# HLLMR/stratum-dsp

Measured on AMD Instinct MI355X. Metric: tracks/sec full analyze_audio(), 3-min 44.1 kHz mono, at 1/2/4/8 MI355X, higher is better.
Workload: dtype f32

## Files before the change

### stratum-dsp_amd/csrc/k_hpcp.hip

```cpp
#include "block_utils.hpp"
#include "kernels.hpp"

namespace sdsp {

constexpr int HP_CW = 16;
constexpr int HPB_CW = HP_CW;
static_assert(HPB_CW == 16, "k_hpcp_band stages a chunk as four 16-byte groups per row");
constexpr int HP_HU = 4;

template <int KCAP>
struct HpcpFrame {
    float e = 0.0f, m1 = 0.0f, m2 = 0.0f;
    float thr = -1.0f;
    float pm[KCAP];
    int pb[KCAP];
    __device__ __forceinline__ void init() {
#pragma unroll
        for (int q = 0; q < KCAP; q++) {
            pm[q] = -1.0f;
            pb[q] = 0;
        }
    }
    template <bool ENERGY = true>
    __device__ __forceinline__ void walk(const float* row, int c0, int cw, const HpcpParams& P) {
        for (int j = 0; j < cw; j++) {
            const int b = c0 + j;
            const float m = row[j];
            if (ENERGY) e += m * m;
            const int c = b - 1;
            if (c >= P.pk_lo && c <= P.pk_hi && !(m1 <= m2 || m1 < m) && m1 > thr) {
                bool gt[KCAP];
#pragma unroll
                for (int q = 0; q < KCAP; q++) gt[q] = m1 > pm[q];
#pragma unroll
                for (int q = KCAP - 1; q >= 1; q--) {
                    const int nbv = gt[q - 1] ? pb[q - 1] : c;
                    pm[q] = __builtin_amdgcn_fmed3f(pm[q], m1, pm[q - 1]);
                    pb[q] = gt[q] ? nbv : pb[q];
                }
                pm[0] = gt[0] ? m1 : pm[0];
                pb[0] = gt[0] ? c : pb[0];
                thr = pm[KCAP - 1];
            }
            m2 = m1;
            m1 = m;
        }
    }
    __device__ __forceinline__ void finish(float (*pc)[HP_FRAMES], int i, const HpcpParams& P,
                                           const HarmEntry* __restrict__ harm, float* __restrict__ chroma,
                                           float* __restrict__ energy, uint64_t g) {
#pragma unroll
        for (int q = 0; q < 12; q++) pc[q][i] = 0.0f;
#pragma unroll
        for (int k = 0; k < KCAP; k++) {
            if (k >= P.K || !(pm[k] > 0.0f)) continue;
            const int bin = pb[k];
            const float xk = sd_maxf(pm[k], 0.0f);
            float w0;
            if (P.p == 0.5f) {
                const float s = __builtin_sqrtf(xk);
                w0 = sd_sqrt_is_powf_half(xk, s) ? s : sd_powf_ool(xk, 0.5f);
            } else {
                w0 = sd_powf_ool(xk, P.p);
            }
            if (w0 <= 0.0f) continue;
            HarmEntry hv[HP_HU];
#pragma unroll
            for (int h = 0; h < HP_HU; h++)
                if (h < P.hmax) hv[h] = harm[bin * HP_HMAX + h];
            bool stop = false;
#pragma unroll
            for (int h = 0; h < HP_HU; h++) {
                if (stop || h >= P.hmax) break;
                const HarmEntry& he = hv[h];
                if (he.state == 0) {
                    stop = true;
                    break;
                }
                if (he.state == 1) continue;
                const float contrib = w0 * he.hw;
                for (int o = 0; o < 3; o++) pc[he.tc[o]][i] += contrib * he.wt[o];
            }
            for (int h = HP_HU + 1; !stop && h <= P.hmax; h++) {
                const HarmEntry he = harm[bin * HP_HMAX + (h - 1)];
                if (he.state == 0) break;
                if (he.state == 1) continue;
                const float contrib = w0 * he.hw;
                for (int o = 0; o < 3; o++) pc[he.tc[o]][i] += contrib * he.wt[o];
            }
        }
        float nsq = 0.0f;
#pragma unroll
        for (int q = 0; q < 12; q++) nsq += pc[q][i] * pc[q][i];
        const float norm = __builtin_sqrtf(nsq);
#pragma unroll
        for (int q = 0; q < 12; q++) {
            float v = pc[q][i];
            if (norm > EPS) v /= norm;
            chroma[g * 12 + q] = v;
        }
        energy[g] = e;
    }
};

template <int KCAP>
__global__ __launch_bounds__(HP_FRAMES) __attribute__((amdgpu_waves_per_eu(4))) void k_hpcp(const float* __restrict__ mags,
                                                    const uint64_t* __restrict__ frame_pfx,
                                                    const uint64_t* __restrict__ tile_pfx,
                                                    const int* __restrict__ tracks, int n_items, HpcpParams P,
                                                    const HarmEntry* __restrict__ harm, float* __restrict__ chroma,
                                                    float* __restrict__ energy) {
    __shared__ float tile[HP_FRAMES][HP_CW + 1];
    __shared__ float pcs[12][HP_FRAMES];
    const uint64_t gb = blockIdx.x;
    const int it = find_track(tile_pfx, n_items, gb);
    const int trk = tracks[it];
    const int64_t F = (int64_t)(frame_pfx[trk + 1] - frame_pfx[trk]);
    const int64_t f0 = (int64_t)(gb - tile_pfx[it]) * HP_FRAMES;
    const int i = threadIdx.x;
    const int64_t f = f0 + i;
    const bool valid = f < F;
    const int lane = i & 63, wrow = i & ~63;
    const int64_t rows = F - f0 < HP_FRAMES ? F - f0 : HP_FRAMES;
    if (wrow >= rows) return;
    const uint64_t g0 = frame_pfx[trk];
    HpcpFrame<KCAP> hf;
    hf.init();
    constexpr int RSTEP = 64 / HP_CW;
    constexpr int NLD = 64 / RSTEP;
    const int sub = lane / HP_CW, jj = lane % HP_CW;
    const float* rowp = mags + (g0 + (uint64_t)f0 + (uint64_t)(wrow + sub)) * (uint64_t)P.stride + jj;
    const uint64_t rstride = (uint64_t)RSTEP * (uint64_t)P.stride;
    float nx[NLD];
    auto load_chunk = [&](int c0) {
        const bool col_ok = c0 + jj < P.B;
#pragma unroll
        for (int u = 0; u < NLD; u++)
            nx[u] = (wrow + sub + u * RSTEP < rows && col_ok) ? rowp[(uint64_t)u * rstride + c0] : 0.0f;
    };
    auto wave_sync = [] {
        __builtin_amdgcn_fence(__ATOMIC_RELEASE, "wavefront");
        __builtin_amdgcn_wave_barrier();
        __builtin_amdgcn_fence(__ATOMIC_ACQUIRE, "wavefront");
    };
    load_chunk(0);
    for (int c0 = 0; c0 < P.B; c0 += HP_CW) {
        wave_sync();
#pragma unroll
        for (int u = 0; u < NLD; u++) tile[wrow + sub + u * RSTEP][jj] = nx[u];
        wave_sync();
        if (c0 + HP_CW < P.B) load_chunk(c0 + HP_CW);
        if (!valid) continue;
        hf.walk(tile[i], c0, P.B - c0 < HP_CW ? P.B - c0 : HP_CW, P);
    }
    if (!valid) return;
    hf.finish(pcs, i, P, harm, chroma, energy, g0 + (uint64_t)f);
}

__device__ float energy_delta(const float* __restrict__ pp, uint64_t total, int n_blocks, int B, float e_blk) {
    if (!(e_blk > 0.0f)) return 0.0f;
    const double u = 0x1p-24, g63 = 63.0 * u / (1.0 - 63.0 * u), g64 = 64.0 * u / (1.0 - 64.0 * u);
    const double gN = (double)B * u / (1.0 - (double)B * u), iu = 1.0 / (1.0 - g63);
    double pu = 0.0, pt = 0.0, eref = 0.0, eo = 0.0;
    for (int g = 0; g < n_blocks; g++) {
        const double bt = (double)pp[(uint64_t)g * total], bu = bt * iu;
        pu += bu;
        pt += bt;
        const int nb = B - 64 * g < 64 ? B - 64 * g : 64;
        eref += __builtin_fmin(bu, (double)nb * u * (1.0 + u) * pu * (1.0 + gN));
        eo += pt;
    }
    const double D = (eref + u * (1.0 + u) * (1.0 + g64) * eo + g63 * pu) * (1.0 + 1e-9);
    const double r = D / (double)e_blk;
    if (!(r < 1.0)) return 1.0f;
    float d = (float)r;
    if ((double)d < r) d = __uint_as_float(__float_as_uint(d) + 1u);
    return d;
}

constexpr float KC_IU_F = (float)(1.0 / (1.0 - 63.0 * 0x1p-24 / (1.0 - 63.0 * 0x1p-24)));
__device__ float energy_delta_f32(float e_blk, float pu, float eref, float eo, const float* __restrict__ pp,
                                  uint64_t total, int n_blocks, int B) {
    if (!(e_blk > 0.0f)) return 0.0f;
    if (!(e_blk >= 0x1p-60f && e_blk <= 0x1p100f)) return energy_delta(pp, total, n_blocks, B, e_blk);
    const float u = 0x1p-24f;
    const float g63 = 63.0f * u / (1.0f - 63.0f * u), g64 = 64.0f * u / (1.0f - 64.0f * u);
    const float D = eref + u * (1.0f + u) * (1.0f + g64) * eo + g63 * pu;
    const float r = (D / e_blk) * (1.0f + 0x1p-14f);
    if (!(r < 1.0f)) return 1.0f;
    return r;
}

template <int KCAP>
__global__ __launch_bounds__(HP_FRAMES) __attribute__((amdgpu_waves_per_eu(4))) void k_hpcp_band(const float* __restrict__ mags,
                                                         const uint64_t* __restrict__ frame_pfx,
                                                         const uint64_t* __restrict__ tile_pfx,
                                                         const int* __restrict__ tracks, int n_items, HpcpParams P,
                                                         const HarmEntry* __restrict__ harm,
                                                         const float* __restrict__ part, int n_blocks, uint64_t total,
                                                         float* __restrict__ chroma, float* __restrict__ energy,
                                                         float* __restrict__ edel) {
    __shared__ float tile[HP_FRAMES][HPB_CW + 1];
    __shared__ float pcs[12][HP_FRAMES];
    const uint64_t gb = blockIdx.x;
    const int it = find_track(tile_pfx, n_items, gb);
    const int trk = tracks[it];
    const int64_t F = (int64_t)(frame_pfx[trk + 1] - frame_pfx[trk]);
    const int64_t f0 = (int64_t)(gb - tile_pfx[it]) * HP_FRAMES;
    const int i = threadIdx.x;
    const int64_t f = f0 + i;
    const bool valid = f < F;
    const int lane = i & 63, wrow = i & ~63;
    const int64_t rows = F - f0 < HP_FRAMES ? F - f0 : HP_FRAMES;
    if (wrow >= rows) return;
    const uint64_t g0 = frame_pfx[trk];
    HpcpFrame<KCAP> hf;
    hf.init();
    if (valid) {
        const float* pp = part + g0 + (uint64_t)f;
        const float u = 0x1p-24f;
        const float gN = (float)P.B * u / (1.0f - (float)P.B * u);
        const float c64 = 64.0f * u * (1.0f + u) * (1.0f + gN);
        const float clast = (float)(P.B - 64 * (n_blocks - 1)) * u * (1.0f + u) * (1.0f + gN);
        float pt = 0.0f, pu = 0.0f, eref = 0.0f, eo = 0.0f;
        for (int g = 0; g < n_blocks; g++) {
            const float bt = pp[(uint64_t)g * total];
            pt += bt;
            const float bu = bt * KC_IU_F;
            pu += bu;
            eref += __builtin_fminf(bu, (g + 1 < n_blocks ? c64 : clast) * pu);
            eo += pt;
        }
        hf.e = pt;
        if (edel) edel[g0 + (uint64_t)f] = energy_delta_f32(pt, pu, eref, eo, pp, total, n_blocks, P.B);
    }
    const int w_lo = P.pk_lo - 1 > 0 ? P.pk_lo - 1 : 0, w_hi = P.pk_hi + 1 < P.B - 1 ? P.pk_hi + 1 : P.B - 1;
    typedef float f4v __attribute__((ext_vector_type(4)));
    const int r4 = lane >> 2, q4 = lane & 3;
    const f4v* rowp4 = reinterpret_cast<const f4v*>(mags + (g0 + (uint64_t)f0 + (uint64_t)(wrow + r4)) * (uint64_t)P.stride + 4 * q4);
    const uint64_t rstride4 = 4 * (uint64_t)P.stride;
    f4v n4[4];
    auto load_chunk = [&](int c0) {
#pragma unroll
        for (int u = 0; u < 4; u++) {
            const int b = c0 + 4 * q4;
            f4v v = {0.0f, 0.0f, 0.0f, 0.0f};
            if (wrow + r4 + 16 * u < rows && b <= w_hi) v = rowp4[(uint64_t)u * rstride4 + (uint64_t)(c0 >> 2)];
            n4[u] = f4v{b <= w_hi ? v.x : 0.0f, b + 1 <= w_hi ? v.y : 0.0f, b + 2 <= w_hi ? v.z : 0.0f,
                        b + 3 <= w_hi ? v.w : 0.0f};
        }
    };
    auto wave_sync = [] {
        __builtin_amdgcn_fence(__ATOMIC_RELEASE, "wavefront");
        __builtin_amdgcn_wave_barrier();
        __builtin_amdgcn_fence(__ATOMIC_ACQUIRE, "wavefront");
    };
    const int c_start = w_lo & ~(HPB_CW - 1);
    if (w_lo <= w_hi) load_chunk(c_start);
    for (int c0 = c_start; c0 <= w_hi; c0 += HPB_CW) {
        wave_sync();
#pragma unroll
        for (int u = 0; u < 4; u++) {
            float* tr = tile[wrow + r4 + 16 * u] + 4 * q4;
            tr[0] = n4[u].x;
            tr[1] = n4[u].y;
            tr[2] = n4[u].z;
            tr[3] = n4[u].w;
        }
        wave_sync();
        if (c0 + HPB_CW <= w_hi) load_chunk(c0 + HPB_CW);
        if (!valid) continue;
        hf.template walk<false>(tile[i], c0, w_hi + 1 - c0 < HPB_CW ? w_hi + 1 - c0 : HPB_CW, P);
    }
    if (!valid) return;
    hf.finish(pcs, i, P, harm, chroma, energy, g0 + (uint64_t)f);
}

void launch_hpcp_band(const float* mags, const uint64_t* frame_pfx, const uint64_t* tile_pfx, const int* tracks,
                      int n_items, uint64_t n_tiles, const HpcpParams& P, const HarmEntry* harm, const float* part,
                      uint64_t total, float* chroma, float* energy, float* edel, hipStream_t st) {
    if (n_tiles == 0) return;
    const int nblk = (P.B + MASK_T - 1) / MASK_T;
    const dim3 grid((unsigned)n_tiles), block(HP_FRAMES);
#define SDSP_HB(K)                                                                                                   \
    hipLaunchKernelGGL(k_hpcp_band<K>, grid, block, 0, st, mags, frame_pfx, tile_pfx, tracks, n_items, P, harm, part, \
                       nblk, total, chroma, energy, edel)
    if (P.K <= 8)
        SDSP_HB(8);
    else if (P.K <= 16)
        SDSP_HB(16);
    else if (P.K <= 24)
        SDSP_HB(24);
    else
        SDSP_HB(HP_KMAX);
#undef SDSP_HB
}
void launch_hpcp(const float* mags, const uint64_t* frame_pfx, const uint64_t* tile_pfx, const int* tracks,
                 int n_items, uint64_t n_tiles, const HpcpParams& P, const HarmEntry* harm, float* chroma,
                 float* energy, hipStream_t st) {
    if (n_tiles == 0) return;
    const dim3 grid((unsigned)n_tiles), block(HP_FRAMES);
    if (P.K <= 8)
        hipLaunchKernelGGL(k_hpcp<8>, grid, block, 0, st, mags, frame_pfx, tile_pfx, tracks, n_items, P, harm, chroma,
                           energy);
    else if (P.K <= 16)
        hipLaunchKernelGGL(k_hpcp<16>, grid, block, 0, st, mags, frame_pfx, tile_pfx, tracks, n_items, P, harm, chroma,
                           energy);
    else if (P.K <= 24)
        hipLaunchKernelGGL(k_hpcp<24>, grid, block, 0, st, mags, frame_pfx, tile_pfx, tracks, n_items, P, harm, chroma,
                           energy);
    else
        hipLaunchKernelGGL(k_hpcp<HP_KMAX>, grid, block, 0, st, mags, frame_pfx, tile_pfx, tracks, n_items, P, harm,
                           chroma, energy);
}

}
```

### stratum-dsp_amd/csrc/k_key_vote.hip

```cpp
#include "block_utils.hpp"
#include "kernels.hpp"

namespace sdsp {

__device__ bool key_raw_near(const float raw[24]) {
    bool near = false;
    for (int m = 0; m < 2; m++) {
        float t1 = 0.0f, t2 = 0.0f;
        for (int k = 0; k < 12; k++) {
            const float v = raw[12 * m + k];
            if (v > t1) {
                t2 = t1;
                t1 = v;
            } else if (v > t2) {
                t2 = v;
            }
        }
        near |= t1 > 0.0f && !(t1 - t2 > KV_NEAR_CONF * t1);
        near |= sd_absf(t1 - 1e-9f) <= KV_NEAR_REL * 1e-9f;
    }
    return near;
}

__device__ void key_from_raw(const float raw[24], float sorted[24], int order[24]) {
// ... 115 lines not shown
    }
    const int best = order[0], tonic = best % 12;
    const bool best_major = best < 12;
    const float p_min3 = avg[(tonic + 3) % 12], p_maj3 = avg[(tonic + 4) % 12];
    const float p_min6 = avg[(tonic + 8) % 12], p_maj6 = avg[(tonic + 9) % 12];
    const float p_min7 = avg[(tonic + 10) % 12], p_maj7 = avg[(tonic + 11) % 12];
    const float margin = sd_maxf(P.mh_margin, 0.0f);
    float minor_score = 0.0f, major_score = 0.0f;
    const float third = sd_absf(p_min3 - p_maj3);
    if (p_min3 > p_maj3 * (1.0f + margin))
        minor_score += third * 2.0f;
    else if (p_maj3 > p_min3 * (1.0f + margin))
        major_score += third * 2.0f;
    const float sixth = sd_absf(p_min6 - p_maj6);
    if (p_min6 > p_maj6 * (1.0f + margin))
        minor_score += sixth * 1.0f;
    else if (p_maj6 > p_min6 * (1.0f + margin))
        major_score += sixth * 1.0f;
    const float seventh = sd_absf(p_min7 - p_maj7);
    if (p_min7 > p_maj7 * (1.0f + margin))
        minor_score += seventh * 1.0f;
    else if (p_maj7 > p_min7 * (1.0f + margin))
        major_score += seventh * 1.0f;
    const float total = minor_score + major_score;
    const bool minor_pref = total > 1e-9f ? minor_score > major_score * (1.0f + margin * 0.5f) : false;
    const bool major_pref = total > 1e-9f ? major_score > minor_score * (1.0f + margin * 0.5f) : false;
    int ch = best;
    if (mode_flip) {
        if (best_major && minor_pref) {
            if (maj_s[tonic] > 0.0f && min_s[tonic] >= maj_s[tonic] * flip_ratio) ch = 12 + tonic;
        } else if (!best_major && major_pref) {
            if (min_s[tonic] > 0.0f && maj_s[tonic] >= min_s[tonic] * flip_ratio) ch = tonic;
        }
    }
    const float cs = ch < 12 ? maj_s[ch] : min_s[ch - 12];
    float other = 0.0f;
    for (int i = 0; i < 24; i++)
        if (order[i] != ch) other = sd_maxf(other, sorted[i]);
    *chosen = ch;
    *conf = cs > 0.0f ? sd_clampf((cs - other) / cs, 0.0f, 1.0f) : 0.0f;
}

constexpr int KV_MAXSCALE = 8;

constexpr double KC_U = 0x1p-24;
constexpr int KC_CAP = 32;
struct KcCand {
    int64_t st;
    int len, w, k;
    float slack;
};
__device__ __forceinline__ float kc_up(double x) {
    float d = (float)x;
    if ((double)d < x) d = __uint_as_float(__float_as_uint(d) + 1u);
    return d;
}
__device__ __forceinline__ double kc_noise(double R, double SS, double K) { return KC_U * (2.0001 * R + (1.0 + K) * SS); }
__device__ __forceinline__ double kc_eta(double d, double p) {
    const double L = p * d / (1.0 - d) + 2.0001 * KC_U * p + 2.0001 * (KC_U + 0x1p-40) + 2.0001 * KC_U;
    return L / (1.0 - L);
}
__device__ __noinline__ int kc_argmax(const float* raw, const float* SS, const float* V, double sf, double K, int64_t st, int len,
                         KcCand* list, int* nlist) {
    int bits = 0;
    for (int m = 0; m < 2; m++) {
        int W = 0;
        for (int k = 1; k < 12; k++)
            if (!(raw[12 * m + k] < raw[12 * m + W])) W = k;
        const double RW = raw[12 * m + W];
        if (!(RW > 0.0)) continue;
        const double NW = kc_noise(RW, SS[12 * m + W] * sf, K), VW = V[12 * m + W] * sf;
        for (int k = 0; k < 12; k++) {
            if (k == W) continue;
            const double Rk = raw[12 * m + k], G = RW - Rk;
            const double need0 = NW + kc_noise(Rk, SS[12 * m + k] * sf, K) + 1.01 * KC_U * RW;
            if (G > need0 + (VW + V[12 * m + k] * sf) * (1.0 + 2.0001 * KC_U)) continue;
            const int q = G > need0 ? atomicAdd(nlist, 1) : KC_CAP;
            if (q < KC_CAP) {
                float sl = (float)(G - need0);
                if ((double)sl > G - need0) sl = __uint_as_float(__float_as_uint(sl) - 1u);
                list[q] = KcCand{st, len, 12 * m + W, 12 * m + k, sl};
            } else {
                bits |= KV_NEAR_ARGMAX;
            }
        }
    }
    return bits;
}
__device__ __noinline__ double kc_clarity(const float* raw, const float* SS, const float* V, double sf, double K, const float* sorted,
                             const int* order, float* beta, int* bits) {
    auto Ax = [&](int x) { return V[x] * sf * (1.0 + 2.0001 * KC_U) + kc_noise(raw[x], SS[x] * sf, K); };
    int Wm[2];
    double AW[2];
    for (int m = 0; m < 2; m++) {
        int W = 0;
        for (int k = 1; k < 12; k++)
            if (!(raw[12 * m + k] < raw[12 * m + W])) W = k;
        Wm[m] = 12 * m + W;
        AW[m] = Ax(Wm[m]);
        if (!(raw[Wm[m]] > 1e-9f) || !((double)raw[Wm[m]] - AW[m] > 0.0)) {
            *bits |= KV_NEAR_RANGE;
            return 1.0;
        }
    }
    double sb = 0.0, bmax = 0.0;
    for (int i = 0; i < 24; i++) {
        const int x = order[i];
        const int W = Wm[x / 12];
        double b = 0.0;
        if (x != W) {
            const double M = raw[W], sc = (double)raw[x] / M, aw = AW[x / 12];
            b = (Ax(x) + sc * aw) / (M - aw) + 2.0001 * KC_U * (sc + (double)sorted[i]);
        }
        beta[x] = kc_up(b);
        sb += b;
        bmax = b > bmax ? b : bmax;
    }
    double srs = 0.0, mn = sorted[0];
    for (int i = 0; i < 24; i++) {
        srs += (double)sorted[i];
        mn = (double)sorted[i] < mn ? (double)sorted[i] : mn;
    }
    const double best = sorted[0], range = best - mn, avg = srs / 24.0, num = best - avg;
    const double dsum = sb + 2.0 * 23.0 * KC_U * srs * 1.01;
    const double davg = dsum / 24.0 + 2.0 * KC_U * __builtin_fabs(avg) * 1.01;
    const double dnum = davg + 2.0 * KC_U * __builtin_fabs(num) * 1.01;
    const double drange = bmax + 2.0 * KC_U * range * 1.01;
    if (!(range - drange > 1e-6)) {
        *bits |= KV_NEAR_RANGE;
        return 1.0;
    }
    const double cl0 = __builtin_fabs(num / range);
    return (dnum + cl0 * drange) / (range - drange) + 2.0 * KC_U * cl0 * 1.01 + 1e-15;
}

#ifndef KV_THREADS
#define KV_THREADS 256
#endif
#ifndef KV_SMALL_ITEMS
#define KV_SMALL_ITEMS 96
#endif
#ifdef SDSP_KV_PROF
#define KV_T(i) do { if (threadIdx.x == 0) kv_t[i] = __builtin_amdgcn_s_memrealtime(); } while (0)
#else
#define KV_T(i) do { } while (0)
#endif
template <int NT>
__global__ __launch_bounds__(NT) __attribute__((amdgpu_waves_per_eu(4))) void k_key_vote(const int* __restrict__ tracks, int n_items,
                                                  const uint64_t* __restrict__ frame_pfx, float* __restrict__ chroma_raw,
                                                  const float* __restrict__ energy, float* __restrict__ chroma_s,
                                                  float* __restrict__ weights, float* __restrict__ seg_scratch,
                                                  const uint64_t* __restrict__ seg_off, const float* __restrict__ tmpl,
                                                  KeyParams P, KeyOut* __restrict__ out, KeyDbg* __restrict__ dbg,
                                                  const float* __restrict__ edel, float* __restrict__ wdel) {
    __shared__ int hist[256];
    __shared__ int misc[4];
    __shared__ int redi[NT / 64];
    __shared__ float acc[48];
    __shared__ int use_w_s, used_s, near_s;
    __shared__ float totw_s;
    __shared__ float tpl[48][12];
    __shared__ int sc_len[KV_MAXSCALE], sc_pfx[KV_MAXSCALE + 1];
    __shared__ float sc_w[KV_MAXSCALE];
    __shared__ KcCand kc_list[KC_CAP];
    __shared__ int kc_n;
    __shared__ unsigned int kc_dmax, kc_emax;
    __shared__ float kc_pa[24], kc_ss[24], kc_v[24];
    __shared__ int kc_w;
    __shared__ double kc_red[NT / 64];
    __shared__ float kc_crs;
    const bool cert = P.near_check && !P.cert_fixed && edel && wdel;
#ifdef SDSP_KV_PROF
    uint64_t kv_t[12] = {};
#endif
    KV_T(0);
    const int it = blockIdx.x;
    const int trk = tracks[it];
    const int64_t F_all = (int64_t)(frame_pfx[trk + 1] - frame_pfx[trk]);
    const uint64_t g0 = frame_pfx[trk];
    float* cr = chroma_raw + g0 * 12;
    for (int k = threadIdx.x; k < 576; k += blockDim.x) tpl[k / 12][k % 12] = tmpl[k];
    if (threadIdx.x == 0) {
        near_s = 0;
        kc_n = 0;
        kc_dmax = 0u;
        kc_emax = 0u;
    }
    if (F_all <= 0) {
        if (threadIdx.x == 0) out[trk] = KeyOut{0, 0, 0.0f, 0.0f, 0, 0, 0, 0};
        return;
    }
    if (P.sharpen > 1.0f) {
        for (int64_t f = threadIdx.x; f < F_all; f += blockDim.x) {
            float* c = cr + f * 12;
            float sq = 0.0f;
            for (int i = 0; i < 12; i++) {
                c[i] = sd_powf(c[i], P.sharpen);
                sq += c[i] * c[i];
            }
            const float nrm = __builtin_sqrtf(sq);
            if (nrm > 1e-10f) {
                for (int i = 0; i < 12; i++) c[i] /= nrm;
            } else {
                const float u = 1.0f / __builtin_sqrtf(12.0f);
                for (int i = 0; i < 12; i++) c[i] = u;
            }
        }
        __syncthreads();
    }
    float* cs_all = chroma_s + g0 * 12;
    auto cx = [](float& a, float& b) {
        const bool sw = b < a;
        const float lo = sw ? b : a, hi = sw ? a : b;
        a = lo;
        b = hi;
    };
    for (int64_t q = threadIdx.x; q < F_all * 12; q += blockDim.x) {
        const int64_t f = (int64_t)((uint32_t)q / 12u);
        const int s = (int)((uint32_t)q - 12u * (uint32_t)f);
        if (F_all > 5 && f >= 2 && f + 2 < F_all) {
            const float* c = cr + (f - 2) * 12 + s;
            float v0 = c[0], v1 = c[12], v2 = c[24], v3 = c[36], v4 = c[48];
#pragma unroll
            for (int r = 0; r < 5; r++) {
                if (r % 2 == 0) {
                    cx(v0, v1);
                    cx(v2, v3);
                } else {
                    cx(v1, v2);
                    cx(v3, v4);
                }
            }
            cs_all[q] = v2;
        } else if (F_all > 5) {
            float v[5];
            int n = 0;
            for (int o = -2; o <= 2; o++) {
                const int64_t fi = f + o;
                if (fi >= 0 && fi < F_all) v[n++] = cr[fi * 12 + s];
            }
            for (int a = 1; a < n; a++) {
                const float x = v[a];
                int b = a;
                while (b > 0 && x < v[b - 1]) {
                    v[b] = v[b - 1];
                    b--;
                }
                v[b] = x;
            }
            cs_all[q] = v[n / 2];
        } else {
            cs_all[q] = cr[q];
        }
    }
    __syncthreads();
    KV_T(1);
    int64_t t0 = 0, F = F_all;
    if (P.edge_trim && F_all >= 200) {
        const float frac = sd_clampf(P.edge_frac, 0.0f, 0.49f);
        const int64_t st = (int64_t)sd_roundf((float)F_all * frac);
        const int64_t en_ = (int64_t)sd_roundf((float)F_all * (1.0f - frac));
        if (en_ > st + 50 && en_ <= F_all) {
            t0 = st;
            F = en_ - st;
        }
    }
    const float* cs = cs_all + t0 * 12;
    const float* en = energy + g0 + t0;
    float* w = weights + g0 + t0;
    const float* ed = cert ? edel + g0 + t0 : nullptr;
    float* wd = cert ? wdel + g0 + t0 : nullptr;
    if (P.weighting) {
        const float med = sd_maxf(block_select_kth(en, (int)F, (int)(F / 2), hist, misc), 1e-12f);
        const float ln12 = sd_logf(12.0f);
        int used_local = 0, rng_local = 0;
        uint32_t dmax_local = 0u, emax_local = 0u;
        for (int64_t f = threadIdx.x; f < F; f += blockDim.x) {
            const float* ch = cs + f * 12;
            float sum = 0.0f;
            for (int k = 0; k < 12; k++) sum += ch[k];
            float tonal = 0.0f;
            if (!(sum <= 1e-12f)) {
                float ent = 0.0f;
                for (int k = 0; k < 12; k++) {
                    const float p = ch[k] / sum;
                    if (p > 1e-12f) ent -= p * sd_logf(p);
                }
                tonal = sd_clampf(1.0f - (ent / ln12), 0.0f, 1.0f);
            }
            if (tonal < P.min_tonal) tonal = 0.0f;
            const float e_norm = sd_maxf(en[f] / med, 0.0f);
            const float wt = sd_powf(tonal, sd_maxf(P.tonal_pow, 0.0f));
            const float we = sd_powf(e_norm, sd_maxf(P.energy_pow, 0.0f));
            const float ww = sd_maxf(wt * we, 0.0f);
            w[f] = ww;
            used_local += ww > 0.0f;
            if (cert) {
                const double d = ed[f];
                const double eta = d < 0.25 ? kc_eta(d, sd_maxf(P.energy_pow, 0.0f)) : 1.0;
                wd[f] = ww > 0.0f ? kc_up(eta * (double)ww) : 0.0f;
                if (!(d < 0.25) || (en[f] > 0.0f && !(e_norm >= 0x1p-100f) && we != 1.0f) ||
                    (ww > 0.0f && !(ww >= 0x1p-100f)) || !(ww < 0x1p100f))
                    rng_local = 1;
                dmax_local = max(dmax_local, __float_as_uint((float)d));
                emax_local = max(emax_local, __float_as_uint(kc_up(eta)));
            }
        }
// ... 268 lines not shown
        int64_t st;
        int len;
        float sw;
        seg_of(q / 24, &st, &len, &sw);
        float* row = S + (size_t)(q / 24) * KV_ROW;
        if (kc2)
            row[q % 24] = wsd3(st, len, toff + q % 24, &row[64 + q % 24], &row[88 + q % 24]);
        else
            row[q % 24] = wsd(st, len, toff + q % 24);
    }
    if (P.mh_on)
        for (int q = threadIdx.x; q < nseg * 13; q += blockDim.x) {
            int64_t st;
            int len;
            float sw;
            seg_of(q / 13, &st, &len, &sw);
            const int i = q % 13;
            S[(size_t)(q / 13) * KV_ROW + (i == 12 ? 51 : 52 + i)] = avg_sum(st, len, i);
        }
    __syncthreads();
    KV_T(3);
    for (int sg = threadIdx.x; sg < nseg; sg += blockDim.x) {
        float* row = S + (size_t)sg * KV_ROW;
        float raw[24], sorted[24];
        int order[24];
        for (int k = 0; k < 24; k++) raw[k] = row[k];
        if (P.near_check && key_raw_near(raw)) atomicOr(&near_s, KV_NEAR_ARGMAX);
        int64_t st;
        int len;
        float sw;
        seg_of(sg, &st, &len, &sw);
        if (kc2) {
            const int b = kc_argmax(raw, row + 64, row + 88, kc_sf(len), kc_K(len), st, len, kc_list, &kc_n) |
                          kc_guard(raw, row + 64, row + 88, kc_sf(len), kc_K(len));
            if (b) atomicOr(&near_s, b);
        }
        key_from_raw(raw, sorted, order);
        if (P.mh_on) {
            int key;
            float conf;
            mode_heuristic(sorted, order, row + 52, row[51], P, &key, &conf);
        }
        const float cl = clarity_of(sorted);
        float kc_dcl = 0.0f;
        if (kc2) {
            float beta[24];
            int b = 0;
            kc_dcl = kc_up(kc_clarity(raw, row + 64, row + 88, kc_sf(len), kc_K(len), sorted, order, beta, &b));
            if (b) atomicOr(&near_s, b);
            for (int k = 0; k < 24; k++) row[64 + k] = beta[k];
            row[112] = kc_dcl;
        }
        for (int k = 0; k < 24; k++) {
            row[k] = sorted[k];
            row[24 + k] = (float)order[k];
        }
        row[48] = cl;
        const float gate = mode == 1 ? P.ms_min_cl : P.min_clarity;
        row[49] = cl >= gate ? 1.0f : 0.0f;
        if (P.near_check && sd_absf(cl - gate) <= sd_maxf(KV_NEAR_CLARITY, kc_dcl))
            atomicOr(&near_s, KV_NEAR_GATE);
        row[50] = cl * sw;
    }
    __syncthreads();
    KV_T(4);
    if (kc2) kc_pair_pass();
    KV_T(5);
    if (threadIdx.x < 24) {
        const int key = threadIdx.x;
        float a = 0.0f;
        double pa = 0.0;
        for (int sg = 0; sg < nseg; sg++) {
            const float* row = S + (size_t)sg * KV_ROW;
            if (row[49] == 0.0f) continue;
            for (int k = 0; k < 24; k++)
                if ((int)row[24 + k] == key) {
                    a += row[k] * row[50];
                    pa += (double)a;
                    break;
                }
        }
        acc[key] = a;
        if (kc2) kc_pa[key] = kc_up(pa);
    }
    if (threadIdx.x == 32) {
        int u = 0;
        float tw = 0.0f;
        for (int sg = 0; sg < nseg; sg++)
            if (S[(size_t)sg * KV_ROW + 49] != 0.0f) {
                u++;
                tw += S[(size_t)sg * KV_ROW + 50];
            }
        used_s = u;
        totw_s = tw;
    }
    __syncthreads();
    KV_T(6);
    const int used = used_s;
    const float totw = totw_s;
    if (used == 0 || (mode == 1 && totw <= 1e-12f)) {
        detect_full(used);
        return;
    }
    if (kc2) {
        if (threadIdx.x == 0) {
            float sorted[24], conf;
            int order[24];
            from_table(acc, sorted, order, &conf);
            kc_w = order[0];
        }
        __syncthreads();
        const int W = kc_w, k = threadIdx.x;
        if (k < 24 && k != W) {
            double D = 0.0;
            bool tie = true;
            for (int sg = 0; sg < nseg; sg++) {
                const float* row = S + (size_t)sg * KV_ROW;
                if (row[49] == 0.0f) continue;
                double rW = 0.0, rK = 0.0;
                for (int j = 0; j < 24; j++) {
                    const int o = (int)row[24 + j];
                    rW = o == W ? (double)row[j] : rW;
                    rK = o == k ? (double)row[j] : rK;
                }
                const double cw = row[50], dc = row[112], bw = row[64 + W], bk = row[64 + k];
                tie = tie && rW == rK && bw == 0.0 && bk == 0.0;
                D += (__builtin_fabs(rW - rK) * dc + (bw + bk) * (cw + dc)) * (1.0 + 4.0001 * KC_U) +
                     2.0001 * KC_U * (rW + rK) * cw;
            }
            D += 2.0001 * KC_U * 1.01 * ((double)kc_pa[W] + (double)kc_pa[k]);
            if (!tie && !((double)acc[W] - (double)acc[k] > D + 1.01 * KC_U * (double)acc[W]))
                atomicOr(&near_s, KV_NEAR_FINAL);
        }
        __syncthreads();
    }
    if (threadIdx.x == 0) {
        float tab[24], sorted[24];
        int order[24];
        for (int k = 0; k < 24; k++) tab[k] = mode == 1 ? acc[k] / totw : acc[k];
        float conf;
        from_table(tab, sorted, order, &conf);
        write_out(order[0], conf, clarity_of(sorted), used);
        put_dbg(sorted, order, order[0]);
    }
    KV_T(7);
#ifdef SDSP_KV_PROF
    if (threadIdx.x == 0 && (blockIdx.x % 64) == 0)
        printf("kvprof blk %d nseg %d smooth %.1f weights %.1f segs %.1f segkey %.1f pair %.1f acc %.1f final %.1f us\n",
               (int)blockIdx.x, nseg, (kv_t[1] - kv_t[0]) * 0.01, (kv_t[2] - kv_t[1]) * 0.01, (kv_t[3] - kv_t[2]) * 0.01,
               (kv_t[4] - kv_t[3]) * 0.01, (kv_t[5] - kv_t[4]) * 0.01, (kv_t[6] - kv_t[5]) * 0.01, (kv_t[7] - kv_t[6]) * 0.01);
#endif
}

void launch_key_vote(const int* tracks, int n_items, const uint64_t* frame_pfx, float* chroma_raw,
                     const float* energy, float* chroma_s, float* weights, float* seg_scratch, const uint64_t* seg_off,
                     const float* tmpl, const KeyParams& P, KeyOut* out, hipStream_t st, KeyDbg* dbg,
                     const float* edel, float* wdel, bool alone) {
    if (n_items == 0) return;
    int cus = 0;
    if (alone && n_items > KV_SMALL_ITEMS) {
        int dev = 0;
        if (hipGetDevice(&dev) != hipSuccess || hipDeviceGetAttribute(&cus, hipDeviceAttributeMultiprocessorCount, dev) != hipSuccess)
            cus = 0;
    }
    if (n_items <= KV_SMALL_ITEMS || (alone && n_items <= cus))
        hipLaunchKernelGGL(k_key_vote<1024>, dim3(n_items), dim3(1024), 0, st, tracks, n_items, frame_pfx, chroma_raw,
                           energy, chroma_s, weights, seg_scratch, seg_off, tmpl, P, out, dbg, edel, wdel);
    else if (alone)
        hipLaunchKernelGGL(k_key_vote<512>, dim3(n_items), dim3(512), 0, st, tracks, n_items, frame_pfx, chroma_raw,
                           energy, chroma_s, weights, seg_scratch, seg_off, tmpl, P, out, dbg, edel, wdel);
    else
        hipLaunchKernelGGL(k_key_vote<KV_THREADS>, dim3(n_items), dim3(KV_THREADS), 0, st, tracks, n_items, frame_pfx,
                           chroma_raw, energy, chroma_s, weights, seg_scratch, seg_off, tmpl, P, out, dbg, edel, wdel);
}

}
```

### stratum-dsp_amd/csrc/k_mask.hip

```cpp
#include "block_utils.hpp"
#include "kernels.hpp"

namespace sdsp {

constexpr int MASK_U = 16;

template <int PW>
__device__ __forceinline__ float mask_pow(float x, float p) {
    if (PW == 2) return x * x;
    if (PW == 1) return x;
    return sd_powf(x, p);
}

template <int PW>
__global__ __launch_bounds__(MASK_T) void k_mask(float* __restrict__ mags, int stride, int B,
                                                  const uint64_t* __restrict__ frame_pfx, const int* __restrict__ tracks,
                                                  int blocks_per_track, int margin, float power, int smooth_only) {
    extern __shared__ float mask_lds[];
    const int it = blockIdx.x / blocks_per_track;
    const int trk = tracks[it];
    const int b = (blockIdx.x % blocks_per_track) * MASK_T + threadIdx.x;
    const int64_t F = (int64_t)(frame_pfx[trk + 1] - frame_pfx[trk]);
    if (b >= B || F <= 0) return;
    float* col = mags + frame_pfx[trk] * (uint64_t)stride + b;
    const int M = margin;
    const int R = 2 * M + 2, RX = M + 1;
    float* pre = mask_lds + threadIdx.x;
    float* raw = mask_lds + (size_t)R * MASK_T + threadIdx.x;
    const float p = sd_maxf(power, 1.0f);
    const float eps = 1e-12f;
    pre[0] = 0.0f;
    float prev = 0.0f;
    int w_slot = 0;
    int s_slot = 0;
    int xw = 0;
    int xr = 0;
    for (int64_t base = 0; base < F + M; base += MASK_U) {
        float xv[MASK_U];
#pragma unroll
        for (int u = 0; u < MASK_U; u++) {
            const int64_t tin = base + u;
            xv[u] = tin < F ? col[tin * stride] : 0.0f;
        }
#pragma unroll
        for (int u = 0; u < MASK_U; u++) {
            const int64_t tin = base + u;
            if (tin >= F + M) break;
            if (tin < F) {
                prev = prev + xv[u];
                w_slot = w_slot + 1 == R ? 0 : w_slot + 1;
                pre[w_slot * MASK_T] = prev;
                raw[xw * MASK_T] = xv[u];
                xw = xw + 1 == RX ? 0 : xw + 1;
            }
            const int64_t t = tin - M;
            if (t < 0) continue;
            const int64_t st = t >= M ? t - M : 0;
            const int64_t en = t + M + 1 < F ? t + M + 1 : F;
            const float denom = (float)(en - st > 1 ? en - st : 1);
            const float x_raw = M == 0 ? xv[u] : raw[xr * MASK_T];
            const float hm = M == 0 ? x_raw : (pre[w_slot * MASK_T] - pre[s_slot * MASK_T]) / denom;
            if (smooth_only) {
                col[t * stride] = hm;
                if (M > 0) xr = xr + 1 == RX ? 0 : xr + 1;
                if (t >= M) s_slot = s_slot + 1 == R ? 0 : s_slot + 1;
                continue;
            }
            const float x = max_bnn(x_raw, 0.0f);
            const float h = max_bnn(hm, 0.0f);
            const float r = max_bnn(x - h, 0.0f);
            const float hp = mask_pow<PW>(h, p);
            const float rp = mask_pow<PW>(r, p);
            const float m = hp / (hp + rp + eps);
            col[t * stride] = x * m;
            if (M > 0) xr = xr + 1 == RX ? 0 : xr + 1;
            if (t >= M) s_slot = s_slot + 1 == R ? 0 : s_slot + 1;
        }
    }
}

template <int M, int PW>
__device__ __forceinline__ float mask_elem(float a, int64_t den, float xr, float p, float inv_w) {
    float hm;
    if (den == 2 * M + 1 && (a == 0.0f || (a >= 0x1p-90f && a <= 0x1p120f))) {
        const float q0 = a * inv_w;
        hm = __builtin_fmaf(__builtin_fmaf(-q0, (float)(2 * M + 1), a), inv_w, q0);
    } else {
        hm = a / (float)(den > 1 ? den : 1);
    }
    const float x = max_bnn(xr, 0.0f);
    const float h = max_bnn(hm, 0.0f);
    const float r = max_bnn(x - h, 0.0f);
    const float hp = mask_pow<PW>(h, p);
    const float rp = mask_pow<PW>(r, p);
    const float m = hp / (hp + rp + 1e-12f);
    return x * m;
}

template <int M, int PW>
__global__ __launch_bounds__(MASK_T) void k_mask_r(float* __restrict__ mags, int stride, int B,
                                                    const uint64_t* __restrict__ frame_pfx,
                                                    const int* __restrict__ tracks, int blocks_per_track,
                                                    float power) {
    constexpr int R = 2 * M + 2, RX = M + 1;
    static_assert(M >= 1 && (2 * M + 1) % 2 == 1 && 2 * M + 1 <= 25, "fast window division validated for 3..25");
    const int it = blockIdx.x / blocks_per_track;
    const int trk = tracks[it];
    const int b = (blockIdx.x % blocks_per_track) * MASK_T + threadIdx.x;
    const int64_t F = (int64_t)(frame_pfx[trk + 1] - frame_pfx[trk]);
    if (b >= B || F <= 0) return;
    float* col = mags + frame_pfx[trk] * (uint64_t)stride + b;
    const float p = sd_maxf(power, 1.0f);
    const float inv_w = 1.0f / (float)(2 * M + 1);
    float P[R], X[RX];
#pragma unroll
    for (int j = 0; j < R; j++) P[j] = 0.0f;
#pragma unroll
    for (int j = 0; j < RX; j++) X[j] = 0.0f;
    float prev = 0.0f;
    auto emit = [&](float a, int64_t den, float xr, int64_t t) {
        __builtin_nontemporal_store(mask_elem<M, PW>(a, den, xr, p, inv_w), &col[t * stride]);
    };
    for (int64_t base = 0; base < F + M; base += R) {
        float xv[R];
        if (base >= 2 * M && base + R <= F) {
#pragma unroll
            for (int u = 0; u < R; u++) xv[u] = __builtin_nontemporal_load(&col[(base + u) * stride]);
#pragma unroll
            for (int u = 0; u < R; u++) {
                prev = prev + xv[u];
                P[(u + 1) % R] = prev;
                X[u % RX] = xv[u];
                emit(P[(u + 1) % R] - P[(u + R - 2 * M) % R], 2 * M + 1, X[(u + 1) % RX], base + u - M);
            }
            continue;
        }
#pragma unroll
        for (int u = 0; u < R; u++) xv[u] = base + u < F ? __builtin_nontemporal_load(&col[(base + u) * stride]) : 0.0f;
#pragma unroll
        for (int u = 0; u < R; u++) {
            const int64_t tin = base + u;
            prev = prev + xv[u];
            P[(u + 1) % R] = prev;
            X[u % RX] = xv[u];
            const int64_t t = tin - M;
            if (t >= 0 && t < F) {
                const int64_t st = t >= M ? t - M : 0;
                const int64_t en = t + M + 1 < F ? t + M + 1 : F;
                emit(P[(u + 1) % R] - P[(u + R - 2 * M) % R], en - st, X[(u + 1) % RX], t);
            }
        }
    }
}

template <int M, int PW>
__global__ __launch_bounds__(MASK_T) __attribute__((amdgpu_waves_per_eu(4, 4))) void k_mask_rp(float* __restrict__ mags, int stride, int B,
                                                     const uint64_t* __restrict__ frame_pfx,
                                                     const int* __restrict__ tracks, int blocks_per_track,
                                                     float power, int st_lo, int st_hi, float* __restrict__ part,
                                                     uint64_t total, int outside) {
    constexpr int R = 2 * M + 2, RX = M + 1;
    static_assert(M >= 1 && 2 * M + 1 <= 25 && R <= MASK_T, "fast window division validated for 3..25");
    __shared__ float tile[R][MASK_T + 1];
    const int it = blockIdx.x / blocks_per_track;
    const int trk = tracks[it];
    const int gblk = blockIdx.x % blocks_per_track;
    const int lane = threadIdx.x;
    const int b = gblk * MASK_T + lane;
    const int64_t F = (int64_t)(frame_pfx[trk + 1] - frame_pfx[trk]);
    if (F <= 0) return;
    if (outside && gblk * MASK_T >= st_lo && gblk * MASK_T + MASK_T - 1 <= st_hi) return;
    const bool live = b < B;
    const bool keep = live && (outside ? (b < st_lo || b > st_hi) : (b >= st_lo && b <= st_hi));
    float* const trk0 = mags + frame_pfx[trk] * (uint64_t)stride;
    const uint32_t lvo = (uint32_t)(live ? b : 0) * 4u;
    const uint32_t lvo_z = live ? (uint32_t)b * 4u : 0x80000000u;
    const uint32_t svo = keep ? (uint32_t)b * 4u : 0x80000000u;
    const uint32_t rowb = (uint32_t)stride * 4u;
    auto row_rsrc = [&](int64_t row, uint32_t bytes) {
        return __builtin_amdgcn_make_buffer_rsrc((void*)(trk0 + row * (int64_t)stride), (short)0, (int)bytes, 0x00020000);
    };
    float* pg = part + (uint64_t)gblk * total + frame_pfx[trk];
    const float p = sd_maxf(power, 1.0f);
    const float inv_w = 1.0f / (float)(2 * M + 1);
    float P[R], X[RX];
#pragma unroll
    for (int j = 0; j < R; j++) P[j] = 0.0f;
#pragma unroll
    for (int j = 0; j < RX; j++) X[j] = 0.0f;
    float prev = 0.0f;
    auto finish = [&](float v, int64_t t, int u) {
        __builtin_amdgcn_raw_buffer_store_b32(__float_as_uint(v), row_rsrc(t, (uint32_t)B * 4u), svo, 0, 2 );
        tile[u][lane] = v * v;
    };
    auto emit_full = [&](float a, float xr, int64_t t, int u, bool chk = true) {
        const float q0 = a * inv_w;
        float hm = __builtin_fmaf(__builtin_fmaf(-q0, (float)(2 * M + 1), a), inv_w, q0);
        const uint32_t ab = __float_as_uint(a);
        const bool bad = ((ab << 1) != 0u) & (ab - 0x12800000u > 0x7B800000u - 0x12800000u);
        if (chk && __builtin_expect(__builtin_amdgcn_ballot_w64(bad) != 0, 0))
            if (bad) hm = a / (float)(2 * M + 1);
        const float x = chk ? max0_quiet(xr) : xr;
        const float h = chk ? max0_quiet(hm) : hm;
        const float r = max_bnn(x - h, 0.0f);
        const float hp = mask_pow<PW>(h, p);
        const float rp = mask_pow<PW>(r, p);
        const float den = hp + rp + 1e-12f;
        if (!chk) {
            const float y = __builtin_amdgcn_rcpf(den);
            const float y1 = __builtin_fmaf(__builtin_fmaf(-den, y, 1.0f), y, y);
            const float q0 = hp * y1;
            finish(x * __builtin_fmaf(__builtin_fmaf(-den, q0, hp), y1, q0), t, u);
            return;
        }
        finish(x * (hp / den), t, u);
    };
    auto fold = [&](int64_t base) {
        __builtin_amdgcn_fence(__ATOMIC_RELEASE, "wavefront");
        __builtin_amdgcn_wave_barrier();
        __builtin_amdgcn_fence(__ATOMIC_ACQUIRE, "wavefront");
        {
            const int fu = lane & 31, hf = lane >> 5;
            const int64_t t = base + fu - M;
            float sum = 0.0f;
            if (fu < R) {
#pragma unroll
                for (int j = 0; j < MASK_T / 2; j++) sum += tile[fu][hf * (MASK_T / 2) + j];
            }
            const float hi = __shfl_down(sum, 32);
            if (hf == 0 && fu < R && t >= 0 && t < F) pg[t] = sum + hi;
        }
        __builtin_amdgcn_fence(__ATOMIC_RELEASE, "wavefront");
        __builtin_amdgcn_wave_barrier();
        __builtin_amdgcn_fence(__ATOMIC_ACQUIRE, "wavefront");
    };
    float xv[R];
    auto load_block = [&](int64_t base) {
        const auto rs = row_rsrc(base, 0x7FFFFFFFu);
        if (base >= 2 * M && base + R <= F) {
#pragma unroll
            for (int u = 0; u < R; u++) xv[u] = __uint_as_float(__builtin_amdgcn_raw_buffer_load_b32(rs, lvo_z, (uint32_t)u * rowb, 2));
        } else {
#pragma unroll
            for (int u = 0; u < R; u++)
                xv[u] = (live && base + u < F) ? __uint_as_float(__builtin_amdgcn_raw_buffer_load_b32(rs, lvo, (uint32_t)u * rowb, 2))
                                               : 0.0f;
        }
    };
    load_block(0);
    for (int64_t base = 0; base < F + M; base += R) {
        if (base >= 2 * M && base + R <= F) {
            uint32_t mb = __float_as_uint(xv[0]);
#pragma unroll
            for (int u = 1; u < R; u++) mb = max(mb, __float_as_uint(xv[u]));
#pragma unroll
            for (int j = 0; j < RX; j++) mb = max(mb, __float_as_uint(X[j]));
            const float mx = __uint_as_float(mb);
            const float pf = prev + xv[0];
            const bool ok = mb < 0x7F800000u && (prev + mx == 0.0f || (pf >= 0x1p-21f && pf >= mx * 0x1p-31f &&
                                                                        prev + (float)R * mx <= 0x1p60f));
            if (__builtin_expect(__builtin_amdgcn_ballot_w64(!ok) == 0, 1)) {
#pragma unroll
                for (int u = 0; u < R; u++) {
                    prev = prev + xv[u];
                    P[(u + 1) % R] = prev;
                    X[u % RX] = xv[u];
                    emit_full(P[(u + 1) % R] - P[(u + R - 2 * M) % R], X[(u + 1) % RX], base + u - M, u, false);
                }
            } else
#pragma unroll
            for (int u = 0; u < R; u++) {
                prev = prev + xv[u];
                P[(u + 1) % R] = prev;
                X[u % RX] = xv[u];
                emit_full(P[(u + 1) % R] - P[(u + R - 2 * M) % R], X[(u + 1) % RX], base + u - M, u);
            }
        } else {
#pragma unroll
            for (int u = 0; u < R; u++) {
                const int64_t tin = base + u;
                prev = prev + xv[u];
                P[(u + 1) % R] = prev;
                X[u % RX] = xv[u];
                const int64_t t = tin - M;
                if (t >= 0 && t < F) {
                    const int64_t st = t >= M ? t - M : 0;
                    const int64_t en = t + M + 1 < F ? t + M + 1 : F;
                    finish(mask_elem<M, PW>(P[(u + 1) % R] - P[(u + R - 2 * M) % R], en - st, X[(u + 1) % RX], p, inv_w),
                           t, u);
                }
            }
        }
        if (base + R < F + M) load_block(base + R);
        fold(base);
    }
}

void launch_mask(float* mags, int stride, int B, const uint64_t* frame_pfx, const int* tracks, int n_items, int margin,
                 float power, hipStream_t st, bool smooth_only) {
    if (n_items == 0) return;
    const int bpt = (B + MASK_T - 1) / MASK_T;
    const size_t lds = (size_t)(2 * margin + 2 + margin + 1) * MASK_T * sizeof(float);
    const float p = sd_maxf(power, 1.0f);
    if (smooth_only) {
        if (margin == 0) return;
        hipLaunchKernelGGL(k_mask<1>, dim3(n_items * bpt), dim3(MASK_T), lds, st, mags, stride, B, frame_pfx, tracks,
                           bpt, margin, power, 1);
        return;
    }
    if (margin == 12 && p == 2.0f) {
        hipLaunchKernelGGL((k_mask_r<12, 2>), dim3(n_items * bpt), dim3(MASK_T), 0, st, mags, stride, B, frame_pfx,
                           tracks, bpt, power);
        return;
    }
    if (p == 2.0f)
        hipLaunchKernelGGL(k_mask<2>, dim3(n_items * bpt), dim3(MASK_T), lds, st, mags, stride, B, frame_pfx, tracks,
                           bpt, margin, power, 0);
    else if (p == 1.0f)
        hipLaunchKernelGGL(k_mask<1>, dim3(n_items * bpt), dim3(MASK_T), lds, st, mags, stride, B, frame_pfx, tracks,
                           bpt, margin, power, 0);
    else
        hipLaunchKernelGGL(k_mask<0>, dim3(n_items * bpt), dim3(MASK_T), lds, st, mags, stride, B, frame_pfx, tracks,
                           bpt, margin, power, 0);
}
bool mask_band_ok(int margin, float power) { return margin == 12 && sd_maxf(power, 1.0f) == 2.0f; }
void launch_mask_band(float* mags, int stride, int B, const uint64_t* frame_pfx, const int* tracks, int n_items,
                      float power, int st_lo, int st_hi, float* part, uint64_t total, hipStream_t st, bool outside) {
    if (n_items == 0) return;
    const int bpt = (B + MASK_T - 1) / MASK_T;
    hipLaunchKernelGGL((k_mask_rp<12, 2>), dim3(n_items * bpt), dim3(MASK_T), 0, st, mags, stride, B, frame_pfx, tracks,
                       bpt, power, st_lo, st_hi, part, total, outside ? 1 : 0);
}

}
```

### stratum-dsp_amd/csrc/kernels.hpp

```cpp
#pragma once

#include <hip/hip_runtime.h>
#include <stdint.h>

#include "sdsp_device.hpp"

namespace sdsp {

constexpr int NVAR = 5;

struct MelChunk {
    uint32_t bits;
    float w0[8], w1[8];
    float bf[8];
};
struct FeatParams {
    int B;
    int stride;
    int K;
    int bs[4], be[4];
    int band_on[4];
    int n_mels;
    const int* chunk_flags;
    const MelChunk* mel_chunks;
// ... 127 lines not shown
constexpr int KV_NEAR_ARGMAX = 1, KV_NEAR_GATE = 2, KV_NEAR_FINAL = 4, KV_NEAR_WSUM = 8;
constexpr int KV_NEAR_RANGE = 16;
struct KeyOut {
    int mode, tonic;
    float conf, clarity;
    int ok;
    int used_segments;
    int weights_used;
    int near;
};

struct TuningParams {
    int stride, lo, hi, step, chf;
    float fres, thr, lim;
};
struct ChromaBin {
    int a, b;
    float w0, w1, w2;
};
struct ChromaParams {
    int B, stride, lo, hi;
    int soft, gate_small;
    int n_log, log_off, bmin;
    float fres, sigma;
};
struct HpcpXParams {
    int B, stride;
    int pk_lo, pk_hi, bk_lo, bk_hi;
    int K, KB, hmax;
    int half, rp, rp_mask, rx, rx_mask;
    int bass, main_ok, bass_ok;
    float p, fres, fmin, fmax, bfmin, bfmax, decay, sigma, bw;
};

struct KeyHpssParams {
    int B, stride, bin0, nb;
    int step, tm, fm;
    float p;
};
constexpr int KH_TILE_FRAMES = 16, KH_TILE_BINS = 64, KH_APPLY_FRAMES = 8;

struct HpssParams {
    int B, stride, m;
};
struct HpssLaunch {
    HpssParams P;
    const float* orig;
    const uint64_t* orig_row0;
    float* h[2];
    float* p[2];
    const uint64_t* row0;
    const uint64_t* fpfx;
    const uint64_t* vtile_pfx;
    uint64_t n_vtiles;
    int* last_it;
    unsigned int* change;
    int n_items;
};
constexpr int HPSS_VM_FRAMES = 32, HPSS_COLS = 256, HPSS_ROW_FRAMES = 256;

struct LegacyParams {
    int sr, hop;
    float min_bpm, max_bpm, res;
    int guard;
    float g[7];
};
struct LegacyOut {
    int ok;
    float bpm, conf;
    int agree;
};
constexpr int LG_COMB_MAX = 2048, LG_AC_MAX = 512;

void launch_peak_gain(const float* x, const uint64_t* in_off, const uint64_t* n_raw, const uint64_t* chunk_pfx, int T,
                      uint64_t n_chunks, unsigned int* chunk_bits, unsigned int* peak_bits, float target, int enable,
                      float* gain, hipStream_t st);
struct LoudnessParams {
    int method;
    float target_rms;
    float target_peak;
    float target_lufs;
    float gate;
    int64_t block;
    float b0, b1, b2, a1, a2;
};
void launch_loudness_gain(const float* x, const uint64_t* in_off, const uint64_t* n_raw, const uint64_t* chunk_pfx,
                          int T, uint64_t n_chunks, unsigned int* chunk_bits, unsigned int* peak_bits,
                          const LoudnessParams& P, float* gain, int* status, hipStream_t st);
void launch_frame_rms(const float* x, const uint64_t* src_off, const float* gain, const uint64_t* n_len,
                      const uint64_t* frame_pfx, int T, uint64_t total, int fs, int hop, float* rms, hipStream_t st, bool per_frame_kernel = false);
void launch_trim(const float* rms, const uint64_t* frame_pfx, int T, const uint64_t* n_raw, int hop, float thr,
                 uint64_t min_frames, int enable, uint64_t* trim_start, uint64_t* trim_end, hipStream_t st,
                 const uint64_t* base_pfx = nullptr, int stride = 1);
void launch_frame_rms_from_raw(const float* raw, const uint64_t* raw_base, const float* x, const uint64_t* src_off,
                               const float* gain, const uint64_t* n_trim, const uint64_t* frame_pfx, int T, uint64_t total,
                               int fs, int hop, float* rms, hipStream_t st);
void launch_energy_onsets(const float* rms, const uint64_t* frame_pfx, const uint64_t* n_trim, int hop, float factor,
                          uint32_t* out, const uint64_t* out_off, int* out_n, int T, hipStream_t st);
void launch_flux_onsets(const float* sfo, const float* hfc, const float* hpe, float* scratch, const uint64_t* frame_pfx,
                        const uint64_t* n_trim, int hop, float pct, uint32_t* out, const uint64_t* out_off,
                        int* out_n, int T, hipStream_t st);
void launch_consensus(const uint32_t* energy, const uint64_t* e_off, const int* e_n, const uint32_t* flux_on,
                      const uint64_t* f_off, const int* f_n, uint64_t kind_stride, int T, uint32_t tol, int enable,
                      const int* has_mags, uint32_t* chosen, const uint64_t* c_off, int* c_n, uint32_t* scratch,
                      hipStream_t st, int hpss = 0);
void launch_features(const RowMap& mags, const uint64_t* frame_pfx, const uint64_t* tile_pfx,
                     int T, uint64_t n_tiles, const FeatParams& P, const MelPlan* mel, float* E, float* H, float* SFX,
                     float* SFO, float* MEL, uint64_t total, hipStream_t st);
void launch_novelty(const float* E, const float* H, const float* SFX, const uint64_t* frame_pfx, int T, uint64_t total,
                    const NovParams& P, float* scratch, float* nov, float* nov_sum, const float* MEL, int n_mels,
                    int mel_k, bool mel_on, unsigned int* mel_max, hipStream_t st);
void launch_fft_tempogram(const int* items, int n_items, int T, const float* nov, const float* nov_sum,
                          const uint64_t* frame_pfx, uint64_t total, const FftTgParams& P, const cx* tw, const cx* rt,
                          cx* gscratch, const uint64_t* out_off, float* out_bpm, float* out_pow, hipStream_t st);
void launch_acf_tempogram(const int* items, int n_items, const float* nov, const uint64_t* frame_pfx, uint64_t total,
                          const float* bpm_grid, const int* lag_grid, int NB, float* out_bpm, float* out_str,
                          hipStream_t st);
void launch_tempo_select(int n_items, const int* active, const float* fft_bpm, const float* fft_pow, const uint64_t* fft_off,
                         const int* fft_k, const float* acf_bpm, const float* acf_str, const uint64_t* acf_off,
                         const SelParams& P, TempoEst* est, float* cand, int cand_cap, hipStream_t st);
void launch_multires(const int* tracks, int n_items, const float* c256, const int* n256, const float* c512,
                     const int* n512, const float* c1024, const int* n1024, int cap256, int cap512, int cap1024,
                     const TempoEst* base_est, const float* nov512, const uint64_t* fpfx512, const MrParams& P,
                     TempoEst* mr_est, int* used, float* final_bpm, float* final_conf, hipStream_t st, MrDbg* dbg = nullptr);
void launch_beat(const int* tracks, int n_items, const uint32_t* onsets, const uint64_t* on_off, const int* on_n,
                 uint32_t sr, const float* bpm, const float* conf, float* scratch, const uint64_t* beat_off,
                 const int* beat_cap, float* beats, float* downs, BeatOut* out, hipStream_t st);
void launch_beat_compact(int n, const BeatOut* out, const uint64_t* beat_off, const float* beats, const float* downs,
                         uint64_t* pfx, float* cb, float* cd, hipStream_t st);
void launch_mask(float* mags, int stride, int B, const uint64_t* frame_pfx, const int* tracks, int n_items, int margin,
                 float power, hipStream_t st, bool smooth_only = false);
void launch_tuning(const float* mags, const uint64_t* frame_pfx, const int* tracks, int n_items, const TuningParams& P,
                   float* out, hipStream_t st);
void launch_chroma(int mode, const float* mags, const uint64_t* frame_pfx, const uint64_t* tile_pfx, const int* tracks,
                   int n_items, uint64_t n_tiles, const ChromaParams& P, const float* tuning, float* chroma,
                   float* energy, hipStream_t st);
void launch_hpcp_x(const float* mags, const uint64_t* frame_pfx, const uint64_t* tile_pfx, const int* tracks,
                   int n_items, uint64_t n_tiles, const HpcpXParams& P, const float* tuning, float* chroma,
                   float* energy, hipStream_t st);
void launch_key_hpss(float* mags, const uint64_t* frame_pfx, const uint64_t* mtile_pfx, uint64_t n_mtiles,
                     const uint64_t* atile_pfx, uint64_t n_atiles, const uint64_t* mask_off, const int* tracks,
                     int n_items, const KeyHpssParams& P, float* mask, hipStream_t st);
void launch_hpss(const HpssLaunch& L, hipStream_t st);
void launch_legacy(const uint32_t* onsets, const uint64_t* on_off, const int* on_n, int n_items, const uint64_t* scr_off,
                   const uint64_t* scr_cap, cx* scratch, const cx* tw, int tw_M, const LegacyParams& P, LegacyOut* out,
                   hipStream_t st);
void launch_hpss_rows(const float* p, const uint64_t* row0, const uint64_t* fpfx, const uint64_t* tile_pfx,
                      uint64_t n_tiles, int n_items, int stride, int B, float* energy, float* fmax, hipStream_t st);
void launch_beat_sync(const int* tracks, int n_items, const uint64_t* frame_pfx, const float* fchroma,
                      const float* fenergy, const float* beats, const uint64_t* beat_off, const uint64_t* row_pfx,
                      float fd, float* chroma, float* energy, hipStream_t st);
bool mask_band_ok(int margin, float power);
void launch_mask_band(float* mags, int stride, int B, const uint64_t* frame_pfx, const int* tracks, int n_items,
                      float power, int st_lo, int st_hi, float* part, uint64_t total, hipStream_t st,
                      bool outside = false);
void launch_hpcp_band(const float* mags, const uint64_t* frame_pfx, const uint64_t* tile_pfx, const int* tracks,
                      int n_items, uint64_t n_tiles, const HpcpParams& P, const HarmEntry* harm, const float* part,
                      uint64_t total, float* chroma, float* energy, float* edel, hipStream_t st);
void launch_hpcp(const float* mags, const uint64_t* frame_pfx, const uint64_t* tile_pfx, const int* tracks,
                 int n_items, uint64_t n_tiles, const HpcpParams& P, const HarmEntry* harm, float* chroma,
                 float* energy, hipStream_t st);
void launch_key_vote(const int* tracks, int n_items, const uint64_t* frame_pfx, float* chroma_raw,
                     const float* energy, float* chroma_s, float* weights, float* seg_scratch, const uint64_t* seg_off,
                     const float* tmpl, const KeyParams& P, KeyOut* out, hipStream_t st, KeyDbg* dbg = nullptr,
                     const float* edel = nullptr, float* wdel = nullptr, bool alone = false);
void launch_synth(float* out, uint64_t n_tracks, uint64_t len, uint32_t sr, const float* bpm, const int* key,
                  uint64_t seed0, hipStream_t st);
void launch_synth_normalize(float* out, uint64_t n_tracks, uint64_t len, unsigned int* peak_bits, hipStream_t st);

}
```

### stratum-dsp_amd/csrc/pipeline.hip

```cpp
#include "pipeline.hpp"

namespace sdsp {

namespace detail {
constexpr int STRIDE2 = 1028;
constexpr int STRIDE8 = 4160;
int base_stride(int fs) {
    if (fs == 2048) return STRIDE2;
    if (fs == 8192) return STRIDE8;
    return (fs / 2 + 1 + 3) & ~3;
}
}

Pipeline::Pipeline(DeviceCtx& d, const sdsp_config& cfg, uint32_t sr, int stages, bool exact_energy, bool key_only,
                   bool nested, bool probe)
    : c_(d),
      d_(d),
      cfg_(cfg),
      sr_(sr),
      bpm_only_(stages == SDSP_STAGES_BPM_ONLY),
      exact_energy_(exact_energy),
      key_only_(key_only),
      nested_(nested || probe),
      fs_((int)std::min<uint64_t>(cfg.frame_size, STFT_GEN_MAX)),
      nb_(fs_ / 2 + 1),
      s2_(base_stride(fs_)),
      kfs_((int)std::min<uint64_t>(key_fft(cfg), STFT_GEN_MAX)),
      khop_((int)std::min<uint64_t>(std::max<uint64_t>(key_hop(cfg), 1), INT32_MAX)),
      ks_(base_stride(kfs_)) {
    if (nested_) c_.pre = probe ? "D." : "X.";
}

void Pipeline::run(const float* d_samples, const std::vector<uint64_t>& in_off, const std::vector<uint64_t>& n_raw,
                   std::vector<TrackRes>& res) {
    const size_t T = n_raw.size();
    res.assign(T, TrackRes{});
    const std::string why = check_supported(cfg_, sr_);
    for (size_t i = 0; i < T; i++) {
        if (n_raw[i] == 0) {
            res[i].status = SDSP_ERR_INVALID_INPUT;
            res[i].err = "Invalid input: Empty audio samples";
        } else if (sr_ == 0) {
            res[i].status = SDSP_ERR_INVALID_INPUT;
            res[i].err = "Invalid input: Invalid sample rate";
        } else if (!why.empty()) {
            res[i].status = SDSP_ERR_NOT_IMPLEMENTED;
            res[i].err = "Not implemented: " + why;
        }
    }
    double budget = 64e9;
    {
        size_t fr = 0, tot = 0;
        if (hipMemGetInfo(&fr, &tot) == hipSuccess) {
            double held = 0;
            for (auto& kv : d_.bufs)
                if (kv.first.compare(0, c_.pre.size(), c_.pre) == 0 && (!c_.pre.empty() || kv.first.compare(0, 2, "X.") != 0))
                    held += (double)kv.second->bytes;
            budget = std::max(4e9, ((double)fr + held) * 0.80 / 1.125);
        }
        if (const double gb = test_hooks().hbm_budget_gb.load(); gb > 0.0) budget = std::max(1.0, gb) * 1e9;
    }
    const uint64_t hop = cfg_.hop_size, khop = (uint64_t)khop_;
    std::vector<int> cur;
    double acc = 0;
    auto flush = [&]() {
        if (!cur.empty()) sub_batch(d_samples, in_off, n_raw, cur, res);
        cur.clear();
        acc = 0;
    };
    times_ = sdsp_stage_times{};
    last_sub_ = false;
    auto t0 = std::chrono::steady_clock::now();
    if (cfg_.enable_normalization && cfg_.normalization != SDSP_NORM_PEAK && why.empty())
        loudness_prepass(d_samples, in_off, n_raw, res);
    std::vector<double> need(T, 0.0);
    double total_need = 0;
    for (size_t i = 0; i < T; i++) {
        if (res[i].status != SDSP_OK) continue;
        const double n = (double)n_raw[i];
        need[i] = n / hop * (s2_ * 4.0 * 1.3 + 4 * 70.0) + (bpm_only_ ? 0.0 : n / khop * ks_ * 4.0) +
                  (n / 256 + n / 1024) * s2_ * 4.0 + 1e6;
        if (cfg_.enable_hpss_onsets || cfg_.enable_tempogram_percussive_fallback)
            need[i] += n / hop * s2_ * 4.0 * 5.0;
        if (cfg_.enable_key_hpss_harmonic && !bpm_only_) need[i] += n / khop * 1024.0 * 4.0;
        if (cfg_.enable_tempogram_multi_resolution && hop != 512) need[i] += n / 512 * s2_ * 4.0 * 1.3;
        total_need += need[i];
    }
    const double parts = std::max(1.0, std::ceil(total_need / budget));
    const double share = total_need / parts;
    double cum = 0;
    int part = 0;
    for (size_t i = 0; i < T; i++) {
        if (res[i].status != SDSP_OK) continue;
        const int p = (int)std::min(parts - 1.0, std::floor((cum + 0.5 * need[i]) / share));
        if (!cur.empty() && (p != part || acc + need[i] > budget)) flush();
        part = p;
        cur.push_back((int)i);
        acc += need[i];
        cum += need[i];
    }
    last_sub_ = true;
    flush();
    last_sub_ = false;
    rerun_tail(finish_key(res, true), res);
    times_.total_ms = std::chrono::duration<double, std::milli>(std::chrono::steady_clock::now() - t0).count();
    times_.key_reruns = reruns_;
    times_.rerun_ms = rerun_ms_;
    d_.last = times_;
    if (!exact_energy_ && !nested_) d_.last_tail_reruns = tail_reruns_;
}

void Pipeline::loudness_prepass(const float* d_samples, const std::vector<uint64_t>& in_off,
                                const std::vector<uint64_t>& n_raw, std::vector<TrackRes>& res) {
    const size_t T = n_raw.size();
    loud_gain_.assign(T, 1.0f);
    loud_stat_.assign(T, 0);
    const LoudnessParams lp = loudness_params(cfg_.normalization, sr_);
    std::vector<uint64_t> off, nr, cpfx(1, 0);
    std::vector<size_t> at;
    for (size_t i = 0; i < T; i++) {
        if (res[i].status != SDSP_OK) continue;
        if (lp.method == 2 && lp.block == 0) {
            res[i].status = SDSP_ERR_INVALID_INPUT;
            res[i].err = "Invalid input: Sample rate too low for LUFS calculation";
            continue;
        }
        at.push_back(i);
        off.push_back(in_off[i]);
        nr.push_back(n_raw[i]);
        cpfx.push_back(cpfx.back() + (n_raw[i] + PK_CH - 1) / PK_CH);
    }
    const int L = (int)at.size();
    if (L == 0) return;
    uint64_t* d_off = c_.up("L.off", off);
    uint64_t* d_nr = c_.up("L.nr", nr);
    uint64_t* d_cpfx = c_.up("L.cpfx", cpfx);
    unsigned int* d_peak = c_.dev<unsigned int>("L.peak", (size_t)L);
    float* d_gain = c_.dev<float>("L.gain", (size_t)L);
    int* d_stat = c_.dev<int>("L.stat", (size_t)L);
    launch_loudness_gain(d_samples, d_off, d_nr, d_cpfx, L, cpfx.back(),
                         c_.dev<unsigned int>("L.peakchunk", std::max<uint64_t>(cpfx.back(), 1)), d_peak, lp, d_gain,
                         d_stat, d_.stream);
    SDSP_HIP_CHECK(hipGetLastError());
    const std::vector<float> g = c_.down(d_gain, (size_t)L);
    const std::vector<int> st = c_.down(d_stat, (size_t)L);
    for (int k = 0; k < L; k++) {
        loud_gain_[at[(size_t)k]] = g[(size_t)k];
        loud_stat_[at[(size_t)k]] = st[(size_t)k];
    }
}

void Pipeline::sub_batch(const float* d_samples, const std::vector<uint64_t>& in_off, const std::vector<uint64_t>& n_raw,
                         const std::vector<int>& idx, std::vector<TrackRes>& res) {
    HostTrace htr;
    Timers tm;
    tm.init(d_);
    tm.mark(0);
    const Front f = front(d_samples, in_off, n_raw, idx, res);
    htr("A");
    tm.mark(1);
    const int NR = (int)f.R.size();
    if (NR == 0) return;
    std::vector<TrackDbg> tdbg(dbg_on() ? (size_t)NR : 0);
    const TempoPassIn bin = base_pass_in(d_samples, f);
    KeyLaunch kl = launch_key(d_samples, bin);
    if (key_only_) {
        join_key_only(kl, f, res);
        htr("E key only");
        return;
    }
    TempoPassOut bo;
    tempo_pass("B.", bin, bo);
    add_pass_times(bo);
    tm.mark(2);
    const std::vector<TempoEst> best = c_.down(bo.est, (size_t)NR);
    const Hpss hp = hpss(bo, best, htr);
    const Onsets on = onsets(d_samples, f, bin, bo, hp);
    htr("B");
    tm.mark(3);
    Tempo tp = seed_tempo(f, best, on, res);
    if (dbg_on() && mr_on()) debug_base(bin, bo, best, tdbg);
    escalate(f, bin, bo, best, tp, tdbg, res);
    htr("C");
    if (perc_on()) {
        perc_fallback(f, bin, bo, best, hp, tp, res);
        htr("C perc");
    }
    if (cfg_.force_legacy_bpm || cfg_.enable_bpm_fusion) legacy_select(f, bin, on, tp, res);
    tm.mark(4);
    if (bpm_only_) {
        for (int i = 0; i < NR; i++) {
            TrackRes& r = res[f.slot[(size_t)i]];
            if (r.status != SDSP_OK) continue;
            r.bpm = tp.fbpm_h[(size_t)i];
            r.bpm_conf = tp.fconf_h[(size_t)i];
        }
        htr("results (bpm only)");
        return;
    }
    const Beats bt = beat_grid(bin, bo, on, tp);
    tm.mark(5);
    std::vector<KeyOut> kout = join_key(d_samples, in_off, n_raw, f, kl, htr, res);
    const ResultsHost rh = download_results(bt, bin, bo);
    htr("D down");
    if (cfg_.enable_key_beat_synchronous && !cfg_.enable_key_log_frequency && !kl.K.empty()) {
        beat_sync_revote(kl, rh, kout);
        htr("E beat-sync");
    }
    times_.beat_ms += tm.ms(4, 5);
    fill_results(f, bin, best, tp, rh, res);
    for (size_t k = 0; k < kout.size(); k++) {
        TrackRes& r = res[f.slot[(size_t)kl.K[k]]];
        if (!kout[k].ok) continue;
        set_key_fields(r, kout[k]);
        r.key_near = kout[k].near;
    }
    if (dbg_on()) {
        debug_key(kl, kout, tdbg);
        for (const TrackDbg& t : tdbg) print_debug(cfg_, t);
    }
    htr("results");
}

Front Pipeline::front(const float* d_samples, const std::vector<uint64_t>& in_off, const std::vector<uint64_t>& n_raw,
                      const std::vector<int>& idx, std::vector<TrackRes>& res) {
    Front f;
    const int T = (int)idx.size();
    const int FS = fs_;
    const int HOP = (int)cfg_.hop_size;
    hipStream_t st = d_.stream;
    std::vector<uint64_t> nr((size_t)T), cpfx((size_t)T + 1, 0), spfx((size_t)T + 1, 0);
    f.off.resize((size_t)T);
    for (int t = 0; t < T; t++) {
        f.off[(size_t)t] = in_off[(size_t)idx[(size_t)t]];
        nr[(size_t)t] = n_raw[(size_t)idx[(size_t)t]];
        cpfx[(size_t)t + 1] = cpfx[(size_t)t] + (nr[(size_t)t] + PK_CH - 1) / PK_CH;
        const uint64_t fs = nr[(size_t)t] >= (uint64_t)FS ? (nr[(size_t)t] - FS) / (FS / 2) + 1 : 1;
        spfx[(size_t)t + 1] = spfx[(size_t)t] + (cfg_.enable_silence_trimming ? fs : 0);
    }
    uint64_t* d_off = c_.up("A.off", f.off);
    uint64_t* d_nr = c_.up("A.nr", nr);
    uint64_t* d_cpfx = c_.up("A.cpfx", cpfx);
    uint64_t* d_spfx = c_.up("A.spfx", spfx);
    unsigned int* d_peak = c_.dev<unsigned int>("A.peak", (size_t)T);
    float* d_gain = c_.dev<float>("A.gain", (size_t)T);
    const float target = sd_powf(10.0f, (0.0f - 1.0f) / 20.0f);
    const bool loud = cfg_.enable_normalization && cfg_.normalization != SDSP_NORM_PEAK;
    std::vector<int> nstat((size_t)T, 0);
    if (loud) {
        std::vector<float> g((size_t)T);
        for (int t = 0; t < T; t++) {
            g[(size_t)t] = loud_gain_[(size_t)idx[(size_t)t]];
            nstat[(size_t)t] = loud_stat_[(size_t)idx[(size_t)t]];
        }
        d_gain = c_.up("A.gain", g);
    } else {
        launch_peak_gain(d_samples, d_off, d_nr, d_cpfx, T, cpfx[(size_t)T],
                         c_.dev<unsigned int>("A.peakchunk", std::max<uint64_t>(cpfx[(size_t)T], 1)), d_peak, target,
                         cfg_.enable_normalization, d_gain, st);
    }
    const int G_e = HOP > 0 && FS % HOP == 0 ? FS / HOP : 0;
    const bool rms_shared = f.rms_shared = cfg_.enable_silence_trimming && HOP > 0 && HOP % 32 == 0 &&
                                           (FS / 2) % HOP == 0 && (G_e == 1 || G_e == 2 || G_e == 4 || G_e == 8);
    std::vector<uint64_t>& rpfx = f.rpfx;
    rpfx.assign((size_t)T + 1, 0);
    for (int t = 0; t < T; t++)
        rpfx[(size_t)t + 1] = rpfx[(size_t)t] + (rms_shared ? (nr[(size_t)t] >= (uint64_t)FS ? (nr[(size_t)t] - FS) / HOP + 1 : 1) : 0);
    uint64_t* d_rpfx = nullptr;
    if (rms_shared) {
        d_rpfx = c_.up("A.rpfx", rpfx);
        f.d_srms = c_.dev<float>("A.rrms", std::max<uint64_t>(rpfx[(size_t)T], 1));
        launch_frame_rms(d_samples, d_off, d_gain, d_nr, d_rpfx, T, rpfx[(size_t)T], FS, HOP, f.d_srms, st);
    } else {
        f.d_srms = c_.dev<float>("A.srms", spfx[(size_t)T]);
        launch_frame_rms(d_samples, d_off, d_gain, d_nr, d_spfx, T, spfx[(size_t)T], FS, FS / 2, f.d_srms, st);
    }
    const float thr = sd_powf(10.0f, cfg_.min_amplitude_db / 20.0f);
    const uint64_t min_samples = sd_f2u64((float)500u / 1000.0f * (float)sr_);
    const uint64_t min_frames = (min_samples + (FS / 2) - 1) / (FS / 2);
    uint64_t* d_ts = c_.dev<uint64_t>("A.ts", (size_t)T);
    uint64_t* d_te = c_.dev<uint64_t>("A.te", (size_t)T);
    launch_trim(f.d_srms, d_spfx, T, d_nr, FS / 2, thr, min_frames, cfg_.enable_silence_trimming, d_ts, d_te, st,
                rms_shared ? d_rpfx : nullptr, rms_shared ? (FS / 2) / HOP : 1);
    SDSP_HIP_CHECK(hipGetLastError());
    f.gain_h = c_.down(d_gain, (size_t)T);
    f.ts = c_.down(d_ts, (size_t)T);
    f.te = c_.down(d_te, (size_t)T);
    for (int t = 0; t < T; t++) {
        TrackRes& r = res[(size_t)idx[(size_t)t]];
        const uint64_t n = f.te[(size_t)t] - f.ts[(size_t)t];
        if (nstat[(size_t)t] != 0) {
            r.status = SDSP_ERR_NUMERICAL;
            r.err = "Numerical error: Mean square too small for LUFS calculation";
            continue;
        }
        if (n == 0) {
            r.status = SDSP_ERR_PROCESSING;
            r.err = "Processing error: Audio is entirely silent after trimming";
            continue;
        }
        r.duration = (float)n / (float)sr_;
        f.R.push_back(t);
        f.slot.push_back((size_t)idx[(size_t)t]);
    }
    return f;
}

TempoPassIn Pipeline::base_pass_in(const float* d_samples, const Front& f) const {
    const int base_top_n =
        (int)std::max<uint64_t>(std::max<uint64_t>(cfg_.tempogram_candidates_top_n, cfg_.tempogram_multi_res_top_k), 10);
    TempoPassIn bin;
    bin.hop = (int)cfg_.hop_size;
    bin.samples = d_samples;
    for (int t : f.R) {
        bin.src_off.push_back(f.off[(size_t)t] + f.ts[(size_t)t]);
        bin.gain_h.push_back(f.gain_h[(size_t)t]);
        bin.n_trim.push_back(f.te[(size_t)t] - f.ts[(size_t)t]);
    }
    bin.top_n = mr_on() ? base_top_n : (cfg_.emit_tempogram_candidates ? (int)cfg_.tempogram_candidates_top_n : 1);
    bin.cand_cap = std::max(bin.top_n, 1);
    bin.gate = mr_on();
    bin.mr_nov = mr_on() && bin.hop == 512;
    return bin;
}

Hpss Pipeline::hpss(const TempoPassOut& bo, const std::vector<TempoEst>& best, HostTrace& htr) {
    Hpss hp;
    if (!hpss_on() && !perc_on()) return hp;
    hipStream_t st = d_.stream;
    std::vector<int> S;
    std::vector<uint64_t> hpfx(1, 0);
    for (size_t i = 0; i < best.size(); i++) {
        const TempoEst& e = best[i];
        if (hpss_on() || (e.ok && e.ambiguous && e.trap_low)) {
            S.push_back((int)i);
            hpfx.push_back(hpfx.back() + (bo.fpfx[i + 1] - bo.fpfx[i]));
        }
    }
    const int NS = (int)S.size();
    const uint64_t totS = hpfx.back();
    if (NS == 0 || totS == 0) return hp;
    std::vector<uint64_t> orow, vt(1, 0), rt(1, 0);
    const uint64_t ncb = (nb_ + HPSS_COLS - 1) / HPSS_COLS;
    for (int k = 0; k < NS; k++) {
        const uint64_t F = hpfx[(size_t)k + 1] - hpfx[(size_t)k];
        orow.push_back(bo.fpfx[(size_t)S[(size_t)k]]);
        vt.push_back(vt.back() + (F + HPSS_VM_FRAMES - 1) / HPSS_VM_FRAMES * ncb);
        rt.push_back(rt.back() + (F + HPSS_ROW_FRAMES - 1) / HPSS_ROW_FRAMES);
    }
    HpssLaunch L{};
    L.P.B = nb_;
    L.P.stride = s2_;
    L.P.m = (int)cfg_.hpss_margin;
    L.orig = bo.mags;
    L.orig_row0 = c_.up("H.orow", orow);
// ... 167 lines not shown
```

### stratum-dsp_amd/csrc/pipeline.hpp

```cpp
#pragma once
#include <algorithm>
#include <chrono>
#include <cmath>
#include <cstdio>
#include <cstdlib>
#include <cstring>
#include <deque>
#include <map>
#include <memory>
#include <string>
#include <vector>

#include "../../include/sdsp_fft_spec.h"
#include "../../include/stratum_hip_debug.h"
#include "kernels.hpp"
#include "sdsp_runtime.hpp"

namespace sdsp {
namespace detail {

int base_stride(int fs);
inline uint64_t key_fft(const sdsp_config& c) {
    return c.enable_key_stft_override ? std::max<uint64_t>(c.key_stft_frame_size, 256) : c.frame_size;
}
// ... 59 lines not shown
        b.ensure(std::max<size_t>(n * sizeof(T), 16));
        return b.as<T>();
    }
    template <class T>
    std::vector<T> down(const T* p, size_t n) {
        std::vector<T> v(n);
        if (n) SDSP_HIP_CHECK(hipMemcpyAsync(v.data(), p, n * sizeof(T), hipMemcpyDeviceToHost, d.stream));
        SDSP_HIP_CHECK(hipStreamSynchronize(d.stream));
        keep.clear();
        return v;
    }
    void sync() {
        SDSP_HIP_CHECK(hipStreamSynchronize(d.stream));
        keep.clear();
    }
};

struct Timers {
    hipEvent_t ev[16];
    int n = 0;
    DeviceCtx* d = nullptr;
    void init(DeviceCtx& dc) {
        d = &dc;
        for (auto& e : ev) SDSP_HIP_CHECK(hipEventCreate(&e));
    }
    void mark(int i, hipStream_t s = nullptr) { SDSP_HIP_CHECK(hipEventRecord(ev[i], s ? s : d->stream)); }
    double ms(int a, int b) {
        float t = 0.0f;
        if (hipEventElapsedTime(&t, ev[a], ev[b]) != hipSuccess) return 0.0;
        return t;
    }
    ~Timers() {
        if (d)
            for (auto& e : ev) (void)hipEventDestroy(e);
    }
};

struct HostTrace {
    bool on = test_hooks().host_trace.load() != 0;
    std::chrono::steady_clock::time_point t0 = std::chrono::steady_clock::now(), tp = t0;
    void operator()(const char* tag) {
        if (!on) return;
        const auto t = std::chrono::steady_clock::now();
        std::fprintf(stderr, "[sdsp host] %-12s +%8.3f ms  (%8.3f)\n", tag,
                     std::chrono::duration<double, std::milli>(t - tp).count(),
                     std::chrono::duration<double, std::milli>(t - t0).count());
        tp = t;
    }
};

struct TrackRes {
    int status = SDSP_OK;
    std::string err;
    float bpm = 0, bpm_conf = 0;
    int key_mode = 0, key_tonic = 0;
    float key_conf = 0, key_clarity = 0, stability = 0, duration = 0;
    float onset_consensus = 0;
    std::vector<float> beats, downs;
    int8_t mr_trig = -1, mr_used = -1, perc_trig = -1, perc_used = -1;
    bool has_cands = false;
    std::vector<sdsp_tempo_candidate> cands;
    int key_near = 0;
    bool key_rerun = false;
};
inline void set_key_fields(TrackRes& r, const KeyOut& ko) {
    r.key_mode = ko.mode;
    r.key_tonic = ko.tonic;
    r.key_conf = ko.conf;
    r.key_clarity = ko.clarity;
}
inline void set_key_fields(TrackRes& r, const TrackRes& rerun) {
    r.key_mode = rerun.key_mode;
    r.key_tonic = rerun.key_tonic;
    r.key_conf = rerun.key_conf;
    r.key_clarity = rerun.key_clarity;
}

struct PassTg {
    int present[NVAR] = {0, 0, 0, 0, 0};
    int NB = 0;
    std::vector<int> items;
    std::vector<uint64_t> fft_off;
    std::vector<int> fft_k;
    std::vector<int> fft_k_track;
    float *acf_bpm = nullptr, *acf_str = nullptr;
    float *fft_bpm = nullptr, *fft_pow = nullptr;
};
struct TempoStageDbg {
    FeatParams fp{};
    PassTg tg;
};

struct TempoPassIn {
    int hop = 0;
    const float* samples = nullptr;
    std::vector<uint64_t> src_off;
    std::vector<float> gain_h;
    std::vector<uint64_t> n_trim;
    int top_n = 0, gate = 0, cand_cap = 0;
    const float* mags_in = nullptr;
    const float* fmax_in = nullptr;
    int reuse = 0;
    const float* base_mags = nullptr;
    const float* base_fmax = nullptr;
    std::vector<uint64_t> base_row0;
    bool mr_nov = false;
    TempoStageDbg* dbg = nullptr;
};
TempoPassIn subset(const TempoPassIn& base, const std::vector<int>& which);
struct TempoPassOut {
    std::vector<uint64_t> fpfx;
    uint64_t total = 0;
    float *mags = nullptr, *fmax = nullptr, *E = nullptr, *H = nullptr, *SFX = nullptr, *SFO = nullptr, *MEL = nullptr,
          *nov = nullptr, *nov_sum = nullptr, *cand = nullptr, *nov_mr = nullptr;
    uint64_t* d_fpfx = nullptr;
    TempoEst* est = nullptr;
    int* active = nullptr;
    std::vector<int> active_h;
    double stft_ms = 0, feat_ms = 0, tempo_ms = 0;
    uint64_t stft_launch = 0;
    uint64_t stft_frames = 0;
    double stft_bytes = 0;
};
struct PassPlan {
    int P_T = 0;
    std::vector<uint64_t> tpfx;
    uint64_t* d_tpfx = nullptr;
    RowMap rm{};
};
struct PassFeat {
    FeatParams fp{};
    bool configured = false, mel_on = false;
};

struct Cand4 {
    float bpm, score, fft, acf;
};
struct TrackDbg {
    bool base = false;
    TempoEst est{};
    std::vector<Cand4> base_c;
    bool mr = false;
    std::vector<Cand4> c256, c512, c1024;
    TempoEst mr_est{};
    MrDbg md{};
    bool key = false;
    KeyOut ko{};
    KeyDbg kd{};
    float tuning = 0.0f;
};
void print_debug(const sdsp_config& c, const TrackDbg& d);

struct KeyTail {
    bool ok = false;
    float* mags8 = nullptr;
    uint64_t* d_kpfx = nullptr;
    std::vector<uint64_t> kpfx{0}, kseg{0};
    float* d_part = nullptr;
    uint64_t total8 = 0;
    int st_lo = 0, st_hi = -1, B8 = 0;
    HpcpParams hp{};
    const HarmEntry* d_ht = nullptr;
    float *d_chroma = nullptr, *d_energy = nullptr, *d_cs = nullptr, *d_w = nullptr, *d_sscr = nullptr;
    const float* d_tpl = nullptr;
    KeyParams kp{};
};
struct KeyPending {
    std::unique_ptr<Timers> kt;
    KeyOut* d_kout = nullptr;
    std::vector<size_t> at;
    KeyTail tail;
};
struct KeyCond {
    HpcpParams hp{};
    bool band = false;
    int st_lo = 0, st_hi = -1;
    float *d_part = nullptr, *d_chroma = nullptr, *d_energy = nullptr, *d_edel = nullptr, *d_tune = nullptr;
    const HarmEntry* d_ht = nullptr;
};

struct Front {
    std::vector<uint64_t> off, ts, te;
    std::vector<float> gain_h;
    std::vector<int> R;
    std::vector<size_t> slot;
    std::vector<uint64_t> rpfx;
    float* d_srms = nullptr;
    bool rms_shared = false;
};
struct KeyLaunch {
    std::vector<int> K;
    std::vector<uint64_t> ktile{0};
    bool serial_streams = false;
    float* d_tune = nullptr;
    uint64_t* d_ktile = nullptr;
    int* d_kid = nullptr;
    KeyOut* d_kout = nullptr;
    KeyDbg* d_kdbg = nullptr;
    KeyTail tail;
    std::unique_ptr<Timers> kt;
};
struct Hpss {
    float *d_P0 = nullptr, *d_hpe = nullptr, *d_hfmax = nullptr;
};
struct Onsets {
    uint32_t* d_chosen = nullptr;
    uint64_t* d_coff = nullptr;
    int* d_cn = nullptr;
    std::vector<int> en_h;
};
struct Tempo {
    std::vector<float> fbpm_h, fconf_h;
    std::vector<int> used, E;
    float *d_fbpm = nullptr, *d_fconf = nullptr;
    int* d_used = nullptr;
    TempoEst* d_mr_all = nullptr;
    std::vector<int> epos;
    std::vector<float> c512_h;
    std::vector<int> n512_own;
    int c512_cap = 0;
    std::vector<std::vector<float>> perc_cands;
    std::vector<uint8_t> perc_took;
};
struct Beats {
    std::vector<uint64_t> boff;
    uint64_t* d_boff = nullptr;
    float *d_beats = nullptr, *d_downs = nullptr;
    BeatOut* d_bout = nullptr;
};
struct ResultsHost {
    std::vector<BeatOut> bout;
    std::vector<uint64_t> bpfx;
    std::vector<float> beats_h, downs_h, cand_h;
    float* d_cbeats = nullptr;
};

}
using namespace detail;

class Pipeline {
   public:
    Pipeline(DeviceCtx& d, const sdsp_config& cfg, uint32_t sr, int stages = SDSP_STAGES_FULL, bool exact_energy = false,
             bool key_only = false, bool nested = false, bool probe = false);
    void debug_tempo_stages(const float* host_mags, const uint64_t* frames, uint64_t n_tracks, int hop,
                            sdsp_debug_tempo_out* out);
    void debug_key_stages(const float* host_mags, const uint64_t* frames, uint64_t n_tracks, int mode, float* masked,
                          float* chroma, float* energy, float* edel, int32_t info[4]);

    void run(const float* d_samples, const std::vector<uint64_t>& in_off, const std::vector<uint64_t>& n_raw,
             std::vector<TrackRes>& res);

   private:
    Ctx c_;
    DeviceCtx& d_;
    const sdsp_config& cfg_;
    uint32_t sr_;
    bool bpm_only_ = false;
    bool exact_energy_ = false;
    bool key_only_ = false;
    bool nested_ = false;
    bool last_sub_ = false;
    uint64_t reruns_ = 0;
    uint64_t tail_reruns_ = 0;
    double rerun_ms_ = 0.0;
    const int fs_, nb_, s2_;
    const int kfs_, khop_, ks_;
    sdsp_stage_times times_{};
    std::vector<float> loud_gain_;
    std::vector<int> loud_stat_;
    std::unique_ptr<KeyPending> key_pending_;
    std::unique_ptr<KeyPending> tail_;
    int sb_parity_ = 0;

    bool tg_on() const { return !cfg_.force_legacy_bpm; }
    bool mr_on() const { return cfg_.enable_tempogram_multi_resolution && tg_on(); }
    bool hpss_on() const { return cfg_.enable_hpss_onsets && cfg_.enable_onset_consensus; }
    bool perc_on() const { return mr_on() && cfg_.enable_tempogram_percussive_fallback; }
    bool dbg_on() const { return cfg_.has_debug_track_id != 0; }
    void add_pass_times(const TempoPassOut& o);

    void loudness_prepass(const float* d_samples, const std::vector<uint64_t>& in_off,
                          const std::vector<uint64_t>& n_raw, std::vector<TrackRes>& res);
    void sub_batch(const float* d_samples, const std::vector<uint64_t>& in_off, const std::vector<uint64_t>& n_raw,
                   const std::vector<int>& idx, std::vector<TrackRes>& res);
    Front front(const float* d_samples, const std::vector<uint64_t>& in_off, const std::vector<uint64_t>& n_raw,
                const std::vector<int>& idx, std::vector<TrackRes>& res);
    TempoPassIn base_pass_in(const float* d_samples, const Front& f) const;
    Hpss hpss(const TempoPassOut& bo, const std::vector<TempoEst>& best, HostTrace& htr);
    Onsets onsets(const float* d_samples, const Front& f, const TempoPassIn& bin, const TempoPassOut& bo, const Hpss& hp);
    Beats beat_grid(const TempoPassIn& bin, const TempoPassOut& bo, const Onsets& on, const Tempo& tp);
    ResultsHost download_results(const Beats& bt, const TempoPassIn& bin, const TempoPassOut& bo);
    void fill_results(const Front& f, const TempoPassIn& bin, const std::vector<TempoEst>& best, const Tempo& tp,
                      const ResultsHost& rh, std::vector<TrackRes>& res);

    void tempo_pass(const std::string& tag, const TempoPassIn& in, TempoPassOut& out);
    PassPlan pass_stft(const std::string& tag, const TempoPassIn& in, TempoPassOut& o, Timers& tm);
    PassFeat pass_features(const std::string& tag, const PassPlan& pl, TempoPassOut& o);
    void pass_novelty(const std::string& tag, const TempoPassIn& in, const PassPlan& pl, const PassFeat& pf,
                      TempoPassOut& o);
    PassTg pass_tempograms(const std::string& tag, const TempoPassIn& in, const PassPlan& pl, const PassFeat& pf,
                           const TempoPassOut& o);
    void pass_select(const std::string& tag, const TempoPassIn& in, const PassPlan& pl, const PassTg& tg,
                     TempoPassOut& o);
    Tempo seed_tempo(const Front& f, const std::vector<TempoEst>& best, const Onsets& on, std::vector<TrackRes>& res);
    void escalate(const Front& f, const TempoPassIn& bin, const TempoPassOut& bo, const std::vector<TempoEst>& best,
                  Tempo& tp, std::vector<TrackDbg>& tdbg, std::vector<TrackRes>& res);
    void perc_fallback(const Front& f, const TempoPassIn& bin, const TempoPassOut& bo, const std::vector<TempoEst>& best,
                       const Hpss& hp, Tempo& tp, std::vector<TrackRes>& res);
    void legacy_select(const Front& f, const TempoPassIn& bin, const Onsets& on, Tempo& tp, std::vector<TrackRes>& res);

    KeyLaunch launch_key(const float* d_samples, const TempoPassIn& bin);
    KeyCond key_condition(const std::string& EP, float* mags8, const std::vector<uint64_t>& kpfx,
                          const std::vector<uint64_t>& ktile, uint64_t* d_kpfx, uint64_t* d_ktile, int* d_kid,
                          hipStream_t st2, Timers& kt);
    void join_key_only(KeyLaunch& kl, const Front& f, std::vector<TrackRes>& res);
    std::vector<KeyOut> join_key(const float* d_samples, const std::vector<uint64_t>& in_off,
                                 const std::vector<uint64_t>& n_raw, const Front& f, KeyLaunch& kl, HostTrace& htr,
                                 std::vector<TrackRes>& res);
    std::vector<size_t> finish_key(std::vector<TrackRes>& res, bool keep_tail = false);
    void rerun_near(const float* d_samples, const std::vector<uint64_t>& in_off, const std::vector<uint64_t>& n_raw,
                    const std::vector<size_t>& near, std::vector<TrackRes>& res);
    void rerun_tail(const std::vector<size_t>& near, std::vector<TrackRes>& res);
    void tail_buffers(KeyTail& t, const KeyCond& kc, float* mags8, uint64_t* d_kpfx, uint64_t total8) const;
    void tail_exact(const KeyTail& t, const int* d_sel, int n, const uint64_t* d_tiles, uint64_t n_tiles, hipStream_t st);
    void beat_sync_revote(const KeyLaunch& kl, const ResultsHost& rh, std::vector<KeyOut>& kout);

    void debug_base(const TempoPassIn& bin, const TempoPassOut& bo, const std::vector<TempoEst>& best,
                    std::vector<TrackDbg>& tdbg);
    void debug_multires(const std::vector<int>& E, bool own512, int cap512, int cap_aux, size_t rows512,
                        const TempoPassOut& o256, const TempoPassOut& b512, const TempoPassOut& o1024,
                        const std::vector<int>& n256, const std::vector<int>& n512, const std::vector<int>& n1024,
                        const TempoEst* d_mr, const MrDbg* d_mdbg, std::vector<TrackDbg>& tdbg);
    void debug_key(const KeyLaunch& kl, const std::vector<KeyOut>& kout, std::vector<TrackDbg>& tdbg);
};

}
```

### stratum-dsp_amd/csrc/pipeline_abi.hip

```cpp
#include <atomic>
#include <condition_variable>
#include <mutex>
#include <thread>

#include "batch_sched.hpp"
#include "pipeline.hpp"

namespace sdsp {
namespace {

std::string fmt2(float v) {
    char b[64];
    std::snprintf(b, sizeof b, "%.2f", (double)v);
    return b;
}

char* dup_str(const std::string& s) {
    char* p = (char*)std::malloc(s.size() + 1);
    std::memcpy(p, s.c_str(), s.size() + 1);
    return p;
}
float* dup_f(const std::vector<float>& v) {
    if (v.empty()) return nullptr;
    float* p = (float*)std::malloc(v.size() * sizeof(float));
// ... 112 lines not shown
}

int32_t run_device(int device, const float* d_samples, const uint64_t* offsets, const uint64_t* lens, uint64_t n,
                   uint32_t sr, const sdsp_config* cfg, void* user_stream, sdsp_result* outs,
                   int stages = SDSP_STAGES_FULL, hipEvent_t wait_ev = nullptr) {
    DeviceCtx& d = device_ctx(device);
    std::lock_guard<std::mutex> lk(d.mu);
    SDSP_HIP_CHECK(hipSetDevice(device));
    return run_locked(d, d_samples, offsets, lens, n, sr, cfg, user_stream, outs, stages, wait_ev);
}

}
}

using namespace sdsp;

namespace sdsp {
namespace {
struct Slot {
    float* d = nullptr;
    uint64_t cap = 0;
    hipEvent_t ready = nullptr;
};
struct DeviceStage {
    int dev = 0;
    hipStream_t copy = nullptr;
    Slot slot[2];
};
std::mutex g_stage_mu;
std::map<int, std::vector<DeviceStage*>>* g_stage_free = new std::map<int, std::vector<DeviceStage*>>();
DeviceStage* stage_acquire(int dev) {
    std::lock_guard<std::mutex> lk(g_stage_mu);
    auto& v = (*g_stage_free)[dev];
    if (!v.empty()) {
        DeviceStage* ds = v.back();
        v.pop_back();
        return ds;
    }
    DeviceStage* ds = new DeviceStage();
    ds->dev = dev;
    return ds;
}
void stage_release(DeviceStage* ds) {
    if (ds->copy) {
        (void)hipSetDevice(ds->dev);
        (void)hipStreamSynchronize(ds->copy);
    }
    std::lock_guard<std::mutex> lk(g_stage_mu);
    (*g_stage_free)[ds->dev].push_back(ds);
}
std::vector<int> device_list_override(int ndev) {
    std::vector<int> devs;
#ifdef SDSP_TEST_HOOKS
    for (int v : test_hooks_devices())
        if (v >= 0 && v < ndev) devs.push_back(v);
#endif
    return devs;
}
}
}

namespace sdsp {
namespace {
template <class F>
int32_t run_stage_probe(const char* name, int32_t device, F f) {
    try {
        DeviceCtx& d = device_ctx(device);
        std::lock_guard<std::mutex> lk(d.mu);
        SDSP_HIP_CHECK(hipSetDevice(device));
        int32_t rc = SDSP_OK;
        try {
            f(d);
        } catch (const std::invalid_argument& e) {
            std::fprintf(stderr, "%s: %s\n", name, e.what());
            rc = SDSP_ERR_INVALID_INPUT;
        } catch (const std::exception& e) {
            std::fprintf(stderr, "%s: %s\n", name, e.what());
            rc = SDSP_ERR_PROCESSING;
        }
        for (hipStream_t s : d.own) (void)hipStreamSynchronize(s);
        for (auto it = d.bufs.begin(); it != d.bufs.end();)
            it = it->first.compare(0, 2, "D.") == 0 ? d.bufs.erase(it) : std::next(it);
        return rc;
    } catch (const std::exception& e) {
        std::fprintf(stderr, "%s: %s\n", name, e.what());
        return SDSP_ERR_PROCESSING;
    }
}
}
}


extern "C" {

int32_t sdsp_analyze_batch_device(const float* d_samples, const uint64_t* offsets, const uint64_t* lens,
                                  uint64_t n_tracks, uint32_t sample_rate, const sdsp_config* cfg, int32_t device,
                                  void* stream, sdsp_result* outs) {
    return sdsp_analyze_batch_device_ex(d_samples, offsets, lens, n_tracks, sample_rate, cfg, device, stream,
                                        SDSP_STAGES_FULL, outs);
}

int32_t sdsp_analyze_batch_device_ex(const float* d_samples, const uint64_t* offsets, const uint64_t* lens,
                                     uint64_t n_tracks, uint32_t sample_rate, const sdsp_config* cfg, int32_t device,
                                     void* stream, int32_t stages, sdsp_result* outs) {
    try {
        return run_device(device, d_samples, offsets, lens, n_tracks, sample_rate, cfg, stream, outs, stages);
    } catch (const std::exception& e) {
        std::fprintf(stderr, "sdsp_analyze_batch_device: %s\n", e.what());
        for (uint64_t i = 0; i < n_tracks; i++) {
            std::memset(&outs[i], 0, sizeof(outs[i]));
            outs[i].status = SDSP_ERR_PROCESSING;
            std::snprintf(outs[i].error_message, sizeof outs[i].error_message, "Processing error: %s", e.what());
        }
        return SDSP_ERR_PROCESSING;
    }
}

int32_t sdsp_debug_key_energy_blocked(const sdsp_config* cfg, uint32_t sample_rate) {
    if (!cfg || sample_rate == 0) return -1;
    return key_energy_blocked(*cfg, sample_rate) ? 1 : 0;
}

int32_t sdsp_debug_last_key_near(int32_t device, uint8_t* out, uint64_t n) {
    try {
        DeviceCtx& d = device_ctx(device);
        std::lock_guard<std::mutex> lk(d.mu);
        for (uint64_t i = 0; i < n; i++) out[i] = i < d.last_near.size() ? d.last_near[(size_t)i] : 0;
        return SDSP_OK;
    } catch (const std::exception&) {
        return SDSP_ERR_PROCESSING;
    }
}

int32_t sdsp_debug_last_tail_reruns(int32_t device, uint64_t* n_tracks) {
    try {
        if (!n_tracks) return SDSP_ERR_INVALID_INPUT;
        DeviceCtx& d = device_ctx(device);
        std::lock_guard<std::mutex> lk(d.mu);
        *n_tracks = d.last_tail_reruns;
        return SDSP_OK;
    } catch (const std::exception&) {
        return SDSP_ERR_PROCESSING;
    }
}

int32_t sdsp_debug_tempo_stages(const float* host_mags, const uint64_t* frames, uint64_t n_tracks, uint32_t sample_rate,
                                uint32_t hop, const sdsp_config* cfg, sdsp_debug_tempo_out* out, int32_t device) {
    if (!host_mags || !frames || !cfg || !out || n_tracks == 0 || n_tracks > (1u << 20) || sample_rate == 0 || hop == 0 ||
        hop > 8192)
        return SDSP_ERR_INVALID_INPUT;
    for (uint64_t t = 0; t < n_tracks; t++)
        if (frames[t] == 0 || frames[t] > (1u << 24)) return SDSP_ERR_INVALID_INPUT;
    return run_stage_probe("sdsp_debug_tempo_stages", device, [&](DeviceCtx& d) {
        Pipeline p(d, *cfg, sample_rate, SDSP_STAGES_FULL, false, false, false, true);
        p.debug_tempo_stages(host_mags, frames, n_tracks, (int)hop, out);
    });
}

int32_t sdsp_debug_key_stages(const float* host_mags, const uint64_t* frames, uint64_t n_tracks, uint32_t sample_rate,
                              const sdsp_config* cfg, int32_t mode, float* masked, float* chroma, float* energy,
                              float* edel, int32_t info[4], int32_t device) {
    if (!host_mags || !frames || !cfg || !masked || !chroma || !energy || !info || n_tracks == 0 ||
        n_tracks > (1u << 20) || sample_rate == 0 || mode < 0 || mode > 2)
        return SDSP_ERR_INVALID_INPUT;
    for (uint64_t t = 0; t < n_tracks; t++)
        if (frames[t] == 0 || frames[t] > (1u << 24)) return SDSP_ERR_INVALID_INPUT;
    return run_stage_probe("sdsp_debug_key_stages", device, [&](DeviceCtx& d) {
        Pipeline p(d, *cfg, sample_rate, SDSP_STAGES_FULL, mode == 2, false, false, true);
        p.debug_key_stages(host_mags, frames, n_tracks, mode, masked, chroma, energy, edel, info);
    });
}

int32_t sdsp_analyze_batch(const float* const* tracks, const uint64_t* lens, uint64_t n_tracks, uint32_t sample_rate,
                           const sdsp_config* cfg, uint32_t device_mask, sdsp_result* outs) {
    std::vector<int> devs;
    int ndev = 0;
    if (hipGetDeviceCount(&ndev) != hipSuccess || ndev <= 0) {
        for (uint64_t i = 0; i < n_tracks; i++) {
            std::memset(&outs[i], 0, sizeof(outs[i]));
            outs[i].status = SDSP_ERR_PROCESSING;
            std::snprintf(outs[i].error_message, sizeof outs[i].error_message, "Processing error: no HIP device");
        }
        return SDSP_ERR_PROCESSING;
    }
    devs = device_list_override(ndev);
    if (devs.empty())
        for (int d = 0; d < ndev && d < 32; d++)
            if (device_mask == 0 ? d == 0 : ((device_mask >> d) & 1u)) devs.push_back(d);
    if (devs.empty()) devs.push_back(0);
    uint64_t max_tracks = 512;
    if (const uint64_t t = test_hooks().batch_chunk_tracks.load()) max_tracks = t;
    const std::vector<uint64_t> cb = plan_chunks(lens, n_tracks, max_tracks, (uint64_t)2 << 30 );
#ifdef SDSP_TEST_HOOKS
    const long fail_chunk = test_hooks().fail_chunk.load();
#endif
    const size_t n_chunks = cb.size() - 1;
    auto mark_failed = [&](size_t c, const std::string& what) {
        for (uint64_t i = cb[c]; i < cb[c + 1]; i++) {
            std::memset(&outs[i], 0, sizeof(outs[i]));
            outs[i].status = SDSP_ERR_PROCESSING;
            std::snprintf(outs[i].error_message, sizeof outs[i].error_message, "Processing error: %s", what.c_str());
        }
    };
    for (size_t c = 0; c < n_chunks; c++) mark_failed(c, "track not analysed");
    std::vector<DeviceStage*> stg;
    std::vector<ChunkDevice> cds;
    for (int dev : devs) {
        stg.push_back(stage_acquire(dev));
        DeviceStage* ds = stg.back();
        ChunkDevice cd;
        cd.stage = [ds, &cb, tracks, lens](int s, size_t c) {
            SDSP_HIP_CHECK(hipSetDevice(ds->dev));
            if (!ds->copy) SDSP_HIP_CHECK(hipStreamCreateWithFlags(&ds->copy, hipStreamNonBlocking));
            Slot& sl = ds->slot[s];
            if (!sl.ready) SDSP_HIP_CHECK(hipEventCreateWithFlags(&sl.ready, hipEventDisableTiming));
            uint64_t tot = 0;
            for (uint64_t i = cb[c]; i < cb[c + 1]; i++) tot += lens[i];
            if (sl.cap < tot) {
                if (sl.d) SDSP_HIP_CHECK(hipFree(sl.d));
                sl.d = nullptr;
                sl.cap = 0;
                const uint64_t want = std::max<uint64_t>(tot + tot / 8, 1);
                SDSP_HIP_CHECK(hipMalloc(&sl.d, want * sizeof(float)));
                note_alloc(want * sizeof(float));
                sl.cap = want;
            }
            uint64_t o = 0;
            for (uint64_t i = cb[c]; i < cb[c + 1]; i++) {
                if (lens[i])
                    SDSP_HIP_CHECK(hipMemcpyAsync(sl.d + o, tracks[i], lens[i] * sizeof(float), hipMemcpyHostToDevice,
                                                  ds->copy));
                o += lens[i];
            }
            SDSP_HIP_CHECK(hipEventRecord(sl.ready, ds->copy));
        };
#ifdef SDSP_TEST_HOOKS
        cd.analyze = [ds, &cb, lens, sample_rate, cfg, outs, fail_chunk](int s, size_t c) {
            if ((long)c == fail_chunk) throw HipError("injected chunk failure (test hook)");
#else
        cd.analyze = [ds, &cb, lens, sample_rate, cfg, outs](int s, size_t c) {
#endif
            const uint64_t a = cb[c], b = cb[c + 1];
            std::vector<uint64_t> off(b - a), ln(b - a);
            uint64_t tot = 0;
            for (uint64_t i = a; i < b; i++) {
                off[i - a] = tot;
                ln[i - a] = lens[i];
                tot += lens[i];
            }
            run_device(ds->dev, ds->slot[s].d, off.data(), ln.data(), b - a, sample_rate, cfg, nullptr, outs + a,
                       SDSP_STAGES_FULL, ds->slot[s].ready);
        };
        cd.drain = [ds]() {
            SDSP_HIP_CHECK(hipSetDevice(ds->dev));
            DeviceCtx& c = device_ctx(ds->dev);
            {
                std::lock_guard<std::mutex> lk(c.mu);
                for (hipStream_t s : c.own) SDSP_HIP_CHECK(hipStreamSynchronize(s));
            }
            if (ds->copy) SDSP_HIP_CHECK(hipStreamSynchronize(ds->copy));
        };
        cds.push_back(cd);
    }
    const size_t failed = run_chunked(n_chunks, cds, [&](size_t c, const std::string& what) {
        std::fprintf(stderr, "sdsp_analyze_batch: %s\n", what.c_str());
        mark_failed(c, what);
    });
    for (DeviceStage* ds : stg) stage_release(ds);
    return failed ? SDSP_ERR_PROCESSING : SDSP_OK;
}

int32_t sdsp_analyze_audio(const float* samples, uint64_t n_samples, uint32_t sample_rate, const sdsp_config* cfg,
                           sdsp_result* out, char* err, uint64_t errlen) {
    std::memset(out, 0, sizeof(*out));
    if (n_samples == 0 || sample_rate == 0) {
        const char* m = n_samples == 0 ? "Invalid input: Empty audio samples" : "Invalid input: Invalid sample rate";
        if (err && errlen) std::snprintf(err, (size_t)errlen, "%s", m);
        out->status = SDSP_ERR_INVALID_INPUT;
        return SDSP_ERR_INVALID_INPUT;
    }
    int32_t rc = SDSP_OK;
    int ndev = 0;
    if (hipGetDeviceCount(&ndev) != hipSuccess || ndev <= 0) {
        out->status = SDSP_ERR_PROCESSING;
        std::snprintf(out->error_message, sizeof out->error_message, "Processing error: no HIP device");
    } else {
        try {
            DeviceCtx& d = device_ctx(0);
            std::lock_guard<std::mutex> lk(d.mu);
            SDSP_HIP_CHECK(hipSetDevice(0));
            DevBuf& in = d.buf("api.track");
            in.ensure(n_samples * sizeof(float));
            SDSP_HIP_CHECK(hipMemcpyAsync(in.p, samples, n_samples * sizeof(float), hipMemcpyHostToDevice, d.stream));
            const uint64_t off = 0;
            rc = run_locked(d, in.as<float>(), &off, &n_samples, 1, sample_rate, cfg, nullptr, out, SDSP_STAGES_FULL,
                            nullptr);
        } catch (const std::exception& e) {
            std::memset(out, 0, sizeof(*out));
            out->status = SDSP_ERR_PROCESSING;
            std::snprintf(out->error_message, sizeof out->error_message, "Processing error: %s", e.what());
        }
    }
    if (rc != SDSP_OK && out->status == SDSP_OK) out->status = rc;
    if (out->status != SDSP_OK) {
        if (err && errlen) std::snprintf(err, (size_t)errlen, "%s", out->error_message);
        const int32_t s = out->status;
        sdsp_result_free(out);
        std::memset(out, 0, sizeof(*out));
        out->status = s;
        return s;
    }
    return SDSP_OK;
}

int32_t sdsp_generate_synthetic(float* d_out, uint64_t n_tracks, uint64_t len, uint32_t sample_rate, uint64_t seed0,
                                int32_t bpm_mode, int32_t device, void* stream, float* bpm_out, int32_t* key_out) {
    try {
        DeviceCtx& d = device_ctx(device);
        std::lock_guard<std::mutex> lk(d.mu);
        SDSP_HIP_CHECK(hipSetDevice(device));
        std::vector<float> bpm((size_t)n_tracks);
// ... 50 lines not shown
```

### stratum-dsp_amd/csrc/pipeline_key.hip

```cpp
#include "pipeline.hpp"

namespace sdsp {

KeyLaunch Pipeline::launch_key(const float* d_samples, const TempoPassIn& bin) {
    KeyLaunch kl;
    KeyTail& t = kl.tail;
    t.kp = key_vote_params(cfg_, false);
    hipStream_t st = d_.stream;
    const int KFS = kfs_, KHOP = khop_;
    std::vector<uint64_t> ksrc;
    std::vector<float> kgain;
    double key_in_bytes = 0;
    for (size_t i = 0; i < bin.n_trim.size(); i++) {
        const uint64_t n = bin.n_trim[i];
        if (bpm_only_) break;
        if (n < (uint64_t)fs_ || n < (uint64_t)KFS) continue;
        const uint64_t F8 = (n - KFS) / (uint64_t)KHOP + 1;
        kl.K.push_back((int)i);
        t.kpfx.push_back(t.kpfx.back() + F8);
        kl.ktile.push_back(kl.ktile.back() + (F8 + HP_FRAMES - 1) / HP_FRAMES);
        t.kseg.push_back(t.kseg.back() + (uint64_t)KV_ROW * seg_rows(t.kp, F8));
        ksrc.push_back(bin.src_off[i]);
        kgain.push_back(bin.gain_h[i]);
        key_in_bytes += 4.0 * (double)n;
    }
    const int NK = (int)kl.K.size();
    kl.kt.reset(new Timers());
    Timers& kt = *kl.kt;
    kt.init(d_);
    sb_parity_ ^= 1;
    const std::string EP = sb_parity_ ? "E1." : "E0.";
    kl.serial_streams = nested_ || test_hooks().serial_streams.load() != 0;
    hipStream_t st2 = kl.serial_streams ? st : d_.stream2;
    hipStream_t st3 = kl.serial_streams ? st : d_.stream3;
    if (NK == 0) return kl;
    const int B8 = KFS / 2 + 1;
    const uint64_t total8 = t.kpfx.back();
    t.d_kpfx = c_.up(EP + "kpfx", t.kpfx);
    kl.d_ktile = c_.up(EP + "ktile", kl.ktile);
    uint64_t* d_kseg = c_.up(EP + "kseg", t.kseg);
    const std::vector<uint64_t> kstr = stft_strips(t.kpfx);
    uint64_t* d_kstr = c_.up(EP + "kstrip", kstr);
    uint64_t* d_ksrc = c_.up(EP + "ksrc", ksrc);
    float* d_kgain = c_.up(EP + "kgain", kgain);
    std::vector<int> kid((size_t)NK);
    for (int k = 0; k < NK; k++) kid[(size_t)k] = k;
    kl.d_kid = c_.up(EP + "kid", kid);
    FftTables& t8 = d_.tables(KFS, true);
    t.mags8 = c_.dev<float>("E.mags8", total8 * ks_);
    kt.mark(7);
    SDSP_HIP_CHECK(hipStreamWaitEvent(st2, kt.ev[7], 0));
    kt.mark(0, st2);
    launch_stft(KFS, false, d_samples, t.d_kpfx, NK, total8, d_ksrc, d_kgain, KHOP, t8.window.as<float>(),
                stft_twp(t8, KFS, false), stft_rtp(t8, KFS, false), t.mags8, t.d_kpfx, ks_, nullptr, st2, d_kstr,
                kstr.back(), c_.dev<uint32_t>("E.redo", total8 + 1));
    SDSP_HIP_CHECK(hipGetLastError());
    kt.mark(1, st2);
    const KeyCond kc = key_condition(EP, t.mags8, t.kpfx, kl.ktile, t.d_kpfx, kl.d_ktile, kl.d_kid, st2, kt);
    kl.d_tune = kc.d_tune;
    std::vector<float> tpl(576);
    key_templates(tpl.data());
    t.d_tpl = c_.up(EP + "tpl", tpl);
    t.kp.near_check = kc.band ? 1 : 0;
    t.kp.cert_fixed = test_hooks().key_cert_fixed.load();
    float* d_cs = c_.dev<float>("E.chroma_s", total8 * 12);
    float* d_w = c_.dev<float>("E.weights", total8);
    float* d_sscr = c_.dev<float>("E.segscr", std::max<uint64_t>(t.kseg.back(), 1));
    kl.d_kout = c_.dev<KeyOut>(EP + "kout", (size_t)NK);
    if (kc.band && kc.d_ht) {
        t.ok = true;
        tail_buffers(t, kc, t.mags8, t.d_kpfx, total8);
        t.d_cs = d_cs;
        t.d_w = d_w;
        t.d_sscr = d_sscr;
    }
    kt.mark(8);
    kt.mark(11, st2);
    SDSP_HIP_CHECK(hipStreamWaitEvent(st3, kt.ev[8], 0));
    SDSP_HIP_CHECK(hipStreamWaitEvent(st3, kt.ev[11], 0));
    kl.d_kdbg = dbg_on() ? c_.dev<KeyDbg>(EP + "kdbg", (size_t)NK) : nullptr;
    float* d_wdel = kc.d_edel ? c_.dev<float>("E.wdel", total8) : nullptr;
    launch_key_vote(kl.d_kid, NK, t.d_kpfx, kc.d_chroma, kc.d_energy, d_cs, d_w, d_sscr, d_kseg, t.d_tpl, t.kp,
                    kl.d_kout, st3, kl.d_kdbg, kc.d_edel, d_wdel, last_sub_ || nested_ || key_only_);
    SDSP_HIP_CHECK(hipGetLastError());
    kt.mark(2, st3);
    if (!nested_) SDSP_HIP_CHECK(hipEventRecord(d_.vote_done, st3));
    times_.stft8192_launches += 1;
    times_.stft8192_frames += total8;
    times_.stft8192_bytes += key_in_bytes + 4.0 * (double)total8 * (double)B8;
    return kl;
}

KeyCond Pipeline::key_condition(const std::string& EP, float* mags8, const std::vector<uint64_t>& kpfx,
                                const std::vector<uint64_t>& ktile, uint64_t* d_kpfx, uint64_t* d_ktile, int* d_kid,
                                hipStream_t st2, Timers& kt) {
    const int NK = (int)kpfx.size() - 1;
    const int KFS = kfs_;
    const int B8 = KFS / 2 + 1;
    const float fres8 = (float)sr_ / (float)KFS;
    const uint64_t total8 = kpfx.back();
    float* d_tune = nullptr;
    const bool use_log = cfg_.enable_key_log_frequency;
    const bool tuned = cfg_.enable_key_tuning_compensation && !use_log;
    const bool whiten = cfg_.enable_key_hpcp_whitening && cfg_.key_hpcp_whitening_smooth_bins >= 3;
    KeyCond kc;
    HpcpParams& hp = kc.hp;
    hp.B = B8;
    hp.stride = ks_;
    key_peak_band(cfg_, sr_, &hp.pk_lo, &hp.pk_hi);
    hp.K = (int)std::max<uint64_t>(cfg_.key_hpcp_peaks_per_frame, 1);
    hp.hmax = (int)std::max<uint64_t>(cfg_.key_hpcp_num_harmonics, 1);
    hp.p = sd_clampf(cfg_.key_hpcp_mag_power, 0.05f, 1.0f);
    const bool blocked = key_energy_blocked(cfg_, sr_);
    const bool band = kc.band = blocked && !exact_energy_;
    float* d_part = kc.d_part = blocked ? c_.dev<float>("E.kpart", total8 * (uint64_t)((B8 + 63) / 64)) : nullptr;
    if (blocked) {
        kc.st_lo = band ? hp.pk_lo - 1 : 0;
        kc.st_hi = band ? hp.pk_hi + 1 : B8 - 1;
        launch_mask_band(mags8, ks_, B8, d_kpfx, d_kid, NK, cfg_.key_harmonic_mask_power, kc.st_lo, kc.st_hi, d_part,
                         total8, st2);
    } else if (cfg_.enable_key_hpss_harmonic) {
        const KeyHpssParams kh = key_hpss_params(cfg_, sr_, B8, fres8, ks_);
        if (kh.nb > 0) {
            std::vector<uint64_t> moff(1, 0), mt(1, 0), at(1, 0);
            for (int k = 0; k < NK; k++) {
                const uint64_t F8 = kpfx[(size_t)k + 1] - kpfx[(size_t)k];
                const uint64_t nds = (F8 + (uint64_t)kh.step - 1) / (uint64_t)kh.step;
                moff.push_back(moff.back() + nds * (uint64_t)kh.nb);
                mt.push_back(mt.back() + ((nds + KH_TILE_FRAMES - 1) / KH_TILE_FRAMES) *
                                             (((uint64_t)kh.nb + KH_TILE_BINS - 1) / KH_TILE_BINS));
                at.push_back(at.back() + (F8 + KH_APPLY_FRAMES - 1) / KH_APPLY_FRAMES);
            }
            uint64_t* d_moff = c_.up(EP + "kh_off", moff);
            uint64_t* d_mt = c_.up(EP + "kh_mt", mt);
            uint64_t* d_at = c_.up(EP + "kh_at", at);
            float* d_kmask = c_.dev<float>("E.kh_mask", std::max<uint64_t>(moff.back(), 1));
            kt.mark(9);
            SDSP_HIP_CHECK(hipStreamWaitEvent(st2, kt.ev[9], 0));
            launch_key_hpss(mags8, d_kpfx, d_mt, mt.back(), d_at, at.back(), d_moff, d_kid, NK, kh, d_kmask, st2);
        }
    } else if (cfg_.enable_key_harmonic_mask)
        launch_mask(mags8, ks_, B8, d_kpfx, d_kid, NK, (int)cfg_.key_spectrogram_smooth_margin,
                    cfg_.key_harmonic_mask_power, st2);
    else if (cfg_.enable_key_spectrogram_time_smoothing)
        launch_mask(mags8, ks_, B8, d_kpfx, d_kid, NK, (int)cfg_.key_spectrogram_smooth_margin,
                    cfg_.key_harmonic_mask_power, st2, true);
    if (tuned) {
        TuningParams tp = tuning_params(cfg_, sr_, B8, fres8, ks_);
        d_tune = kc.d_tune = c_.dev<float>("E.tune", (size_t)NK);
        launch_tuning(mags8, d_kpfx, d_kid, NK, tp, d_tune, st2);
        SDSP_HIP_CHECK(hipGetLastError());
    }
    float* d_chroma = kc.d_chroma = c_.dev<float>("E.chroma", total8 * 12);
    float* d_energy = kc.d_energy = c_.dev<float>("E.energy", total8);
    float* d_edel = nullptr;
    if (!nested_) SDSP_HIP_CHECK(hipStreamWaitEvent(st2, d_.vote_done, 0));
    if (use_log) {
        const ChromaParams cp = chroma_params(cfg_, sr_, 1, B8, fres8, ks_);
        launch_chroma(1, mags8, d_kpfx, d_ktile, d_kid, NK, ktile.back(), cp, nullptr, d_chroma, d_energy, st2);
    } else if (cfg_.enable_key_hpcp && (d_tune || whiten || cfg_.enable_key_hpcp_bass_blend)) {
        const HpcpXParams hx = hpcp_x_params(cfg_, sr_, B8, fres8, whiten, ks_);
        launch_hpcp_x(mags8, d_kpfx, d_ktile, d_kid, NK, ktile.back(), hx, d_tune, d_chroma, d_energy, st2);
    } else if (cfg_.enable_key_hpcp) {
        std::vector<HarmEntry> ht =
            harm_table(B8, sr_, KFS, cfg_.soft_mapping_sigma, hp.hmax, cfg_.key_hpcp_harmonic_decay);
        HarmEntry* d_ht = c_.up(EP + "harm", ht);
        kc.d_ht = d_ht;
        kt.mark(10);
        SDSP_HIP_CHECK(hipStreamWaitEvent(st2, kt.ev[10], 0));
        if (band) {
            d_edel = kc.d_edel = c_.dev<float>("E.edel", total8);
            launch_hpcp_band(mags8, d_kpfx, d_ktile, d_kid, NK, ktile.back(), hp, d_ht, d_part, total8, d_chroma,
                             d_energy, d_edel, st2);
        }
        else
            launch_hpcp(mags8, d_kpfx, d_ktile, d_kid, NK, ktile.back(), hp, d_ht, d_chroma, d_energy, st2);
    } else {
        const ChromaParams cp = chroma_params(cfg_, sr_, 0, B8, fres8, ks_);
        launch_chroma(0, mags8, d_kpfx, d_ktile, d_kid, NK, ktile.back(), cp, d_tune, d_chroma, d_energy, st2);
    }
    SDSP_HIP_CHECK(hipGetLastError());
    return kc;
}

void Pipeline::join_key_only(KeyLaunch& kl, const Front& f, std::vector<TrackRes>& res) {
    if (kl.K.empty()) return;
    SDSP_HIP_CHECK(hipStreamWaitEvent(d_.stream, kl.kt->ev[2], 0));
    const std::vector<KeyOut> ko = c_.down(kl.d_kout, kl.K.size());
    for (size_t k = 0; k < kl.K.size(); k++)
        if (ko[k].ok) set_key_fields(res[f.slot[(size_t)kl.K[k]]], ko[k]);
}

std::vector<KeyOut> Pipeline::join_key(const float* d_samples, const std::vector<uint64_t>& in_off,
                                       const std::vector<uint64_t>& n_raw, const Front& f, KeyLaunch& kl,
                                       HostTrace& htr, std::vector<TrackRes>& res) {
    rerun_near(d_samples, in_off, n_raw, finish_key(res), res);
    std::vector<KeyOut> kout;
    const size_t NK = kl.K.size();
    const bool beat_sync = cfg_.enable_key_beat_synchronous && !cfg_.enable_key_log_frequency;
    const bool defer_key =
        NK > 0 && !beat_sync && !kl.serial_streams && !dbg_on() && test_hooks().no_key_defer.load() == 0;
    if (defer_key) {
        key_pending_.reset(new KeyPending());
        key_pending_->kt = std::move(kl.kt);
        key_pending_->d_kout = kl.d_kout;
        for (int i : kl.K) key_pending_->at.push_back(f.slot[(size_t)i]);
        key_pending_->tail = std::move(kl.tail);
    } else if (NK > 0) {
        SDSP_HIP_CHECK(hipStreamWaitEvent(d_.stream, kl.kt->ev[2], 0));
        kout = c_.down(kl.d_kout, NK);
        htr("E join");
        times_.stft8192_ms += kl.kt->ms(0, 1);
        times_.key_ms += kl.kt->ms(1, 2);
    }
    return kout;
}

std::vector<size_t> Pipeline::finish_key(std::vector<TrackRes>& res, bool keep_tail) {
    std::vector<size_t> near;
    if (!key_pending_) return near;
    std::unique_ptr<KeyPending> kp = std::move(key_pending_);
    SDSP_HIP_CHECK(hipStreamWaitEvent(d_.stream, kp->kt->ev[2], 0));
    const std::vector<KeyOut> kout = c_.down(kp->d_kout, kp->at.size());
    for (size_t k = 0; k < kp->at.size(); k++) {
        TrackRes& r = res[kp->at[k]];
        const KeyOut& ko = kout[k];
        if (!ko.ok) continue;
        set_key_fields(r, ko);
        r.key_near = ko.near;
        if (ko.near) near.push_back(kp->at[k]);
    }
    times_.stft8192_ms += kp->kt->ms(0, 1);
    times_.key_ms += kp->kt->ms(1, 2);
    if (keep_tail && kp->tail.ok) tail_ = std::move(kp);
    return near;
}

void Pipeline::rerun_tail(const std::vector<size_t>& near_all, std::vector<TrackRes>& res) {
    std::unique_ptr<KeyPending> kp = std::move(tail_);
    if (near_all.empty() || !kp || exact_energy_ || nested_) return;
    const KeyTail& t = kp->tail;
    const auto t0 = std::chrono::steady_clock::now();
    std::vector<size_t> near;
    for (size_t i : near_all)
        if (res[i].status == SDSP_OK) near.push_back(i);
    if (near.empty()) return;
    std::vector<int> sel;
    for (size_t i : near)
        for (size_t k = 0; k < kp->at.size(); k++)
            if (kp->at[k] == i) sel.push_back((int)k);
    if (sel.size() != near.size()) throw HipError("rerun_tail: a near track is not in the last sub-batch");
    const int n = (int)sel.size();
    std::vector<uint64_t> tp(1, 0), sp(1, 0);
    for (int k : sel) {
        const uint64_t F = t.kpfx[(size_t)k + 1] - t.kpfx[(size_t)k];
        tp.push_back(tp.back() + (F + HP_FRAMES - 1) / HP_FRAMES);
        sp.push_back(sp.back() + (t.kseg[(size_t)k + 1] - t.kseg[(size_t)k]));
    }
    hipStream_t st = d_.stream;
    int* d_sel = c_.up("E.tail_sel", sel);
    uint64_t* d_tp = c_.up("E.tail_tile", tp);
    uint64_t* d_sp = c_.up("E.tail_seg", sp);
    tail_exact(t, d_sel, n, d_tp, tp.back(), st);
    KeyParams kx = t.kp;
    kx.near_check = 0;
    launch_key_vote(d_sel, n, t.d_kpfx, t.d_chroma, t.d_energy, t.d_cs, t.d_w, t.d_sscr, d_sp, t.d_tpl, kx, kp->d_kout,
                    st, nullptr, nullptr, nullptr, true);
    SDSP_HIP_CHECK(hipGetLastError());
    const std::vector<KeyOut> ko = c_.down(kp->d_kout, kp->at.size());
    for (int j = 0; j < n; j++) {
        TrackRes& r = res[near[(size_t)j]];
        const KeyOut& o = ko[(size_t)sel[(size_t)j]];
        if (!o.ok) {
            r.status = SDSP_ERR_PROCESSING;
            r.err = "Processing error: key certification rerun failed (no key from the exact energies)";
            r.key_rerun = true;
            continue;
        }
        set_key_fields(r, o);
        r.key_rerun = true;
    }
    reruns_ += (uint64_t)n;
    tail_reruns_ += (uint64_t)n;
    rerun_ms_ += std::chrono::duration<double, std::milli>(std::chrono::steady_clock::now() - t0).count();
}

void Pipeline::tail_exact(const KeyTail& t, const int* d_sel, int n, const uint64_t* d_tiles, uint64_t n_tiles,
                          hipStream_t st) {
    launch_mask_band(t.mags8, ks_, t.B8, t.d_kpfx, d_sel, n, cfg_.key_harmonic_mask_power, t.st_lo, t.st_hi, t.d_part,
                     t.total8, st, true);
    SDSP_HIP_CHECK(hipGetLastError());
    launch_hpcp(t.mags8, t.d_kpfx, d_tiles, d_sel, n, n_tiles, t.hp, t.d_ht, t.d_chroma, t.d_energy, st);
    SDSP_HIP_CHECK(hipGetLastError());
}

void Pipeline::rerun_near(const float* d_samples, const std::vector<uint64_t>& in_off, const std::vector<uint64_t>& n_raw,
                          const std::vector<size_t>& near, std::vector<TrackRes>& res) {
    if (near.empty() || exact_energy_ || nested_) return;
    std::vector<uint64_t> o2, l2;
    for (size_t i : near) o2.push_back(in_off[i]), l2.push_back(n_raw[i]);
    std::vector<TrackRes> r2;
    Pipeline px(d_, cfg_, sr_, SDSP_STAGES_FULL, true, true, true);
    px.run(d_samples, o2, l2, r2);
    for (size_t j = 0; j < near.size(); j++) {
        TrackRes& r = res[near[j]];
        if (r2[j].status != SDSP_OK) {
            r.status = SDSP_ERR_PROCESSING;
            r.err = "Processing error: key certification rerun failed (" + r2[j].err + ")";
            continue;
        }
        set_key_fields(r, r2[j]);
        r.key_rerun = true;
    }
    reruns_ += near.size();
    rerun_ms_ += d_.last.total_ms;
}

void Pipeline::tail_buffers(KeyTail& t, const KeyCond& kc, float* mags8, uint64_t* d_kpfx, uint64_t total8) const {
    t.mags8 = mags8;
    t.d_kpfx = d_kpfx;
    t.d_part = kc.d_part;
    t.total8 = total8;
    t.st_lo = kc.st_lo;
    t.st_hi = kc.st_hi;
    t.B8 = kc.hp.B;
    t.hp = kc.hp;
    t.d_ht = kc.d_ht;
    t.d_chroma = kc.d_chroma;
    t.d_energy = kc.d_energy;
}

void Pipeline::beat_sync_revote(const KeyLaunch& kl, const ResultsHost& rh, std::vector<KeyOut>& kout) {
    hipStream_t st = d_.stream;
    const int NK = (int)kl.K.size();
    std::vector<int> sel, sel_id;
    std::vector<uint64_t> sb_off, rpfx(1, 0), sseg(1, 0);
    for (int k = 0; k < NK; k++) {
        const int i = kl.K[(size_t)k];
        const int nb = rh.bout[(size_t)i].ok > 0 ? rh.bout[(size_t)i].n_beats : 0;
        if (nb < 1) continue;
        sel.push_back(k);
        sel_id.push_back((int)sel_id.size());
        sb_off.push_back(rh.bpfx[(size_t)i]);
        const uint64_t rows = (uint64_t)nb - 1;
        rpfx.push_back(rpfx.back() + rows);
        sseg.push_back(sseg.back() + (uint64_t)KV_ROW * seg_rows(kl.tail.kp, rows));
    }
    const int NS = (int)sel.size();
    if (NS == 0) return;
    const uint64_t total8 = kl.tail.kpfx.back();
    ChromaParams cp = chroma_params(cfg_, sr_, 0, kfs_ / 2 + 1, (float)sr_ / (float)kfs_, ks_);
    cp.gate_small = 0;
    float* fc = c_.dev<float>("E.bs_fc", total8 * 12);
    float* fe = c_.dev<float>("E.bs_fe", total8);
    launch_chroma(0, kl.tail.mags8, kl.tail.d_kpfx, kl.d_ktile, kl.d_kid, NK, kl.ktile.back(), cp, kl.d_tune, fc, fe, st);
    int* d_sel = c_.up("E.bs_sel", sel);
    int* d_sid = c_.up("E.bs_id", sel_id);
    uint64_t* d_sboff = c_.up("E.bs_boff", sb_off);
    uint64_t* d_rpfx = c_.up("E.bs_rpfx", rpfx);
    uint64_t* d_sseg = c_.up("E.bs_seg", sseg);
    const uint64_t rows = std::max<uint64_t>(rpfx.back(), 1);
    float* bc = c_.dev<float>("E.bs_chroma", rows * 12);
    float* be = c_.dev<float>("E.bs_energy", rows);
    const float fd = (float)khop_ / (float)sr_;
    launch_beat_sync(d_sel, NS, kl.tail.d_kpfx, fc, fe, rh.d_cbeats, d_sboff, d_rpfx, fd, bc, be, st);
    float* bcs = c_.dev<float>("E.bs_chroma_s", rows * 12);
    float* bw = c_.dev<float>("E.bs_weights", rows);
    float* bscr = c_.dev<float>("E.bs_segscr", std::max<uint64_t>(sseg.back(), 1));
    KeyOut* d_bko = c_.dev<KeyOut>("E.bs_kout", (size_t)NS);
    launch_key_vote(d_sid, NS, d_rpfx, bc, be, bcs, bw, bscr, d_sseg, kl.tail.d_tpl, kl.tail.kp, d_bko, st);
    SDSP_HIP_CHECK(hipGetLastError());
    std::vector<KeyOut> bko = c_.down(d_bko, (size_t)NS);
    for (int j = 0; j < NS; j++) kout[(size_t)sel[(size_t)j]] = bko[(size_t)j];
}

}
```

Measured before the change: 3016.

## Move near-key certification rerun onto the GPU with device-side selection

Replaces the host-driven near-track key rerun, which downloaded results, selected tracks on the host, uploaded index arrays and relaunched, or spun up a nested pipeline, with a device-side selection kernel. That kernel compacts near tracks and their tile and segment prefixes. The mask, HPCP and key-vote kernels are then launched over the full grid and early-exit blocks beyond a device-resident live count. Key work is split into halves with separate timers so the rerun can run in-stream without host round trips. The costs are launching full-size grids that mostly exit early, and a more complex pipeline state.

```diff
diff --git a/stratum-dsp_amd/csrc/k_hpcp.hip b/stratum-dsp_amd/csrc/k_hpcp.hip
--- a/stratum-dsp_amd/csrc/k_hpcp.hip
+++ b/stratum-dsp_amd/csrc/k_hpcp.hip
@@ -109,10 +109,12 @@
                                                     const uint64_t* __restrict__ tile_pfx,
                                                     const int* __restrict__ tracks, int n_items, HpcpParams P,
                                                     const HarmEntry* __restrict__ harm, float* __restrict__ chroma,
-                                                    float* __restrict__ energy) {
+                                                    float* __restrict__ energy,
+                                                    const uint64_t* __restrict__ n_tiles_live) {
     __shared__ float tile[HP_FRAMES][HP_CW + 1];
     __shared__ float pcs[12][HP_FRAMES];
     const uint64_t gb = blockIdx.x;
+    if (n_tiles_live && gb >= *n_tiles_live) return;
     const int it = find_track(tile_pfx, n_items, gb);
     const int trk = tracks[it];
     const int64_t F = (int64_t)(frame_pfx[trk + 1] - frame_pfx[trk]);
@@ -297,21 +299,21 @@
 }
 void launch_hpcp(const float* mags, const uint64_t* frame_pfx, const uint64_t* tile_pfx, const int* tracks,
                  int n_items, uint64_t n_tiles, const HpcpParams& P, const HarmEntry* harm, float* chroma,
-                 float* energy, hipStream_t st) {
+                 float* energy, hipStream_t st, const uint64_t* n_tiles_live) {
     if (n_tiles == 0) return;
     const dim3 grid((unsigned)n_tiles), block(HP_FRAMES);
     if (P.K <= 8)
         hipLaunchKernelGGL(k_hpcp<8>, grid, block, 0, st, mags, frame_pfx, tile_pfx, tracks, n_items, P, harm, chroma,
-                           energy);
+                           energy, n_tiles_live);
     else if (P.K <= 16)
         hipLaunchKernelGGL(k_hpcp<16>, grid, block, 0, st, mags, frame_pfx, tile_pfx, tracks, n_items, P, harm, chroma,
-                           energy);
+                           energy, n_tiles_live);
     else if (P.K <= 24)
         hipLaunchKernelGGL(k_hpcp<24>, grid, block, 0, st, mags, frame_pfx, tile_pfx, tracks, n_items, P, harm, chroma,
-                           energy);
+                           energy, n_tiles_live);
     else
         hipLaunchKernelGGL(k_hpcp<HP_KMAX>, grid, block, 0, st, mags, frame_pfx, tile_pfx, tracks, n_items, P, harm,
-                           chroma, energy);
-}
-
-}
+                           chroma, energy, n_tiles_live);
+}
+
+}
diff --git a/stratum-dsp_amd/csrc/k_key_vote.hip b/stratum-dsp_amd/csrc/k_key_vote.hip
--- a/stratum-dsp_amd/csrc/k_key_vote.hip
+++ b/stratum-dsp_amd/csrc/k_key_vote.hip
@@ -291,7 +291,9 @@
                                                   float* __restrict__ weights, float* __restrict__ seg_scratch,
                                                   const uint64_t* __restrict__ seg_off, const float* __restrict__ tmpl,
                                                   KeyParams P, KeyOut* __restrict__ out, KeyDbg* __restrict__ dbg,
-                                                  const float* __restrict__ edel, float* __restrict__ wdel) {
+                                                  const float* __restrict__ edel, float* __restrict__ wdel,
+                                                  const int* __restrict__ n_live) {
+    if (n_live && (int)blockIdx.x >= *n_live) return;
     __shared__ int hist[256];
     __shared__ int misc[4];
     __shared__ int redi[NT / 64];
@@ -866,11 +868,75 @@
 #endif
 }
 
+constexpr int KS_T = 256;
+__global__ __launch_bounds__(KS_T) void k_key_near_select(const int* __restrict__ tracks, int n,
+                                                          const KeyOut* __restrict__ out,
+                                                          const uint64_t* __restrict__ frame_pfx,
+                                                          const uint64_t* __restrict__ seg_pfx, int* __restrict__ sel,
+                                                          int* __restrict__ count, uint64_t* __restrict__ tile_pfx,
+                                                          uint64_t* __restrict__ seg_off) {
+    __shared__ int s_cnt[KS_T];
+    __shared__ uint32_t s_til[KS_T];
+    const int tid = threadIdx.x;
+    int cnt = 0;
+    uint64_t tiles = 0;
+    for (int c0 = 0; c0 < n; c0 += KS_T) {
+        const int i = c0 + tid;
+        int trk = 0, flag = 0;
+        uint32_t tl = 0;
+        if (i < n) {
+            trk = tracks[i];
+            flag = out[trk].ok != 0 && out[trk].near != 0;
+            if (flag) tl = (uint32_t)((frame_pfx[trk + 1] - frame_pfx[trk] + HP_FRAMES - 1) / HP_FRAMES);
+        }
+        s_cnt[tid] = flag;
+        s_til[tid] = tl;
+        __syncthreads();
+        for (int d = 1; d < KS_T; d <<= 1) {
+            const int c = tid >= d ? s_cnt[tid - d] : 0;
+            const uint32_t t = tid >= d ? s_til[tid - d] : 0u;
+            __syncthreads();
+            s_cnt[tid] += c;
+            s_til[tid] += t;
+            __syncthreads();
+        }
+        if (flag) {
+            const int pos = cnt + s_cnt[tid] - 1;
+            sel[pos] = trk;
+            tile_pfx[pos] = tiles + (uint64_t)(s_til[tid] - tl);
+            seg_off[pos] = seg_pfx[trk];
+        }
+        cnt += s_cnt[KS_T - 1];
+        tiles += (uint64_t)s_til[KS_T - 1];
+        __syncthreads();
+    }
+    for (int j = cnt + tid; j <= n; j += KS_T) tile_pfx[j] = tiles;
+    if (tid == 0) *count = cnt;
+}
+
+void launch_key_near_select(const int* tracks, int n, const KeyOut* out, const uint64_t* frame_pfx,
+                            const uint64_t* seg_pfx, int* sel, int* count, uint64_t* tile_pfx, uint64_t* seg_off,
+                            hipStream_t st) {
+    if (n == 0) return;
+    hipLaunchKernelGGL(k_key_near_select, dim3(1), dim3(KS_T), 0, st, tracks, n, out, frame_pfx, seg_pfx, sel, count,
+                       tile_pfx, seg_off);
+}
 void launch_key_vote(const int* tracks, int n_items, const uint64_t* frame_pfx, float* chroma_raw,
                      const float* energy, float* chroma_s, float* weights, float* seg_scratch, const uint64_t* seg_off,
                      const float* tmpl, const KeyParams& P, KeyOut* out, hipStream_t st, KeyDbg* dbg,
-                     const float* edel, float* wdel, bool alone) {
+                     const float* edel, float* wdel, bool alone, const int* n_live) {
     if (n_items == 0) return;
+    if (n_live) {
+        if (alone)
+            hipLaunchKernelGGL(k_key_vote<1024>, dim3(n_items), dim3(1024), 0, st, tracks, n_items, frame_pfx,
+                               chroma_raw, energy, chroma_s, weights, seg_scratch, seg_off, tmpl, P, out, dbg, edel, wdel,
+                               n_live);
+        else
+            hipLaunchKernelGGL(k_key_vote<KV_THREADS>, dim3(n_items), dim3(KV_THREADS), 0, st, tracks, n_items,
+                               frame_pfx, chroma_raw, energy, chroma_s, weights, seg_scratch, seg_off, tmpl, P, out, dbg,
+                               edel, wdel, n_live);
+        return;
+    }
     int cus = 0;
     if (alone && n_items > KV_SMALL_ITEMS) {
         int dev = 0;
@@ -879,13 +945,14 @@
     }
     if (n_items <= KV_SMALL_ITEMS || (alone && n_items <= cus))
         hipLaunchKernelGGL(k_key_vote<1024>, dim3(n_items), dim3(1024), 0, st, tracks, n_items, frame_pfx, chroma_raw,
-                           energy, chroma_s, weights, seg_scratch, seg_off, tmpl, P, out, dbg, edel, wdel);
+                           energy, chroma_s, weights, seg_scratch, seg_off, tmpl, P, out, dbg, edel, wdel, n_live);
     else if (alone)
         hipLaunchKernelGGL(k_key_vote<512>, dim3(n_items), dim3(512), 0, st, tracks, n_items, frame_pfx, chroma_raw,
-                           energy, chroma_s, weights, seg_scratch, seg_off, tmpl, P, out, dbg, edel, wdel);
+                           energy, chroma_s, weights, seg_scratch, seg_off, tmpl, P, out, dbg, edel, wdel, n_live);
     else
         hipLaunchKernelGGL(k_key_vote<KV_THREADS>, dim3(n_items), dim3(KV_THREADS), 0, st, tracks, n_items, frame_pfx,
-                           chroma_raw, energy, chroma_s, weights, seg_scratch, seg_off, tmpl, P, out, dbg, edel, wdel);
-}
-
-}
+                           chroma_raw, energy, chroma_s, weights, seg_scratch, seg_off, tmpl, P, out, dbg, edel, wdel,
+                           n_live);
+}
+
+}
diff --git a/stratum-dsp_amd/csrc/k_mask.hip b/stratum-dsp_amd/csrc/k_mask.hip
--- a/stratum-dsp_amd/csrc/k_mask.hip
+++ b/stratum-dsp_amd/csrc/k_mask.hip
@@ -153,16 +153,18 @@
     }
 }
 
-template <int M, int PW>
+template <int M, int PW, bool OUTSIDE>
 __global__ __launch_bounds__(MASK_T) __attribute__((amdgpu_waves_per_eu(4, 4))) void k_mask_rp(float* __restrict__ mags, int stride, int B,
                                                      const uint64_t* __restrict__ frame_pfx,
                                                      const int* __restrict__ tracks, int blocks_per_track,
                                                      float power, int st_lo, int st_hi, float* __restrict__ part,
-                                                     uint64_t total, int outside) {
+                                                     uint64_t total, const int* __restrict__ n_live) {
+    constexpr int outside = OUTSIDE ? 1 : 0;
     constexpr int R = 2 * M + 2, RX = M + 1;
     static_assert(M >= 1 && 2 * M + 1 <= 25 && R <= MASK_T, "fast window division validated for 3..25");
     __shared__ float tile[R][MASK_T + 1];
     const int it = blockIdx.x / blocks_per_track;
+    if (OUTSIDE && n_live && it >= *n_live) return;
     const int trk = tracks[it];
     const int gblk = blockIdx.x % blocks_per_track;
     const int lane = threadIdx.x;
@@ -180,7 +182,7 @@
     auto row_rsrc = [&](int64_t row, uint32_t bytes) {
         return __builtin_amdgcn_make_buffer_rsrc((void*)(trk0 + row * (int64_t)stride), (short)0, (int)bytes, 0x00020000);
     };
-    float* pg = part + (uint64_t)gblk * total + frame_pfx[trk];
+    float* pg = OUTSIDE ? nullptr : part + (uint64_t)gblk * total + frame_pfx[trk];
     const float p = sd_maxf(power, 1.0f);
     const float inv_w = 1.0f / (float)(2 * M + 1);
     float P[R], X[RX];
@@ -191,7 +193,7 @@
     float prev = 0.0f;
     auto finish = [&](float v, int64_t t, int u) {
         __builtin_amdgcn_raw_buffer_store_b32(__float_as_uint(v), row_rsrc(t, (uint32_t)B * 4u), svo, 0, 2 );
-        tile[u][lane] = v * v;
+        if (!OUTSIDE) tile[u][lane] = v * v;
     };
     auto emit_full = [&](float a, float xr, int64_t t, int u, bool chk = true) {
         const float q0 = a * inv_w;
@@ -292,7 +294,7 @@
             }
         }
         if (base + R < F + M) load_block(base + R);
-        fold(base);
+        if (!OUTSIDE) fold(base);
     }
 }
 
@@ -325,11 +327,18 @@
 }
 bool mask_band_ok(int margin, float power) { return margin == 12 && sd_maxf(power, 1.0f) == 2.0f; }
 void launch_mask_band(float* mags, int stride, int B, const uint64_t* frame_pfx, const int* tracks, int n_items,
-                      float power, int st_lo, int st_hi, float* part, uint64_t total, hipStream_t st, bool outside) {
+                      float power, int st_lo, int st_hi, float* part, uint64_t total, hipStream_t st) {
     if (n_items == 0) return;
     const int bpt = (B + MASK_T - 1) / MASK_T;
-    hipLaunchKernelGGL((k_mask_rp<12, 2>), dim3(n_items * bpt), dim3(MASK_T), 0, st, mags, stride, B, frame_pfx, tracks,
-                       bpt, power, st_lo, st_hi, part, total, outside ? 1 : 0);
-}
-
-}
+    hipLaunchKernelGGL((k_mask_rp<12, 2, false>), dim3(n_items * bpt), dim3(MASK_T), 0, st, mags, stride, B, frame_pfx,
+                       tracks, bpt, power, st_lo, st_hi, part, total, (const int*)nullptr);
+}
+void launch_mask_outside(float* mags, int stride, int B, const uint64_t* frame_pfx, const int* tracks, int n_items,
+                         float power, int st_lo, int st_hi, hipStream_t st, const int* n_live) {
+    if (n_items == 0) return;
+    const int bpt = (B + MASK_T - 1) / MASK_T;
+    hipLaunchKernelGGL((k_mask_rp<12, 2, true>), dim3(n_items * bpt), dim3(MASK_T), 0, st, mags, stride, B, frame_pfx,
+                       tracks, bpt, power, st_lo, st_hi, (float*)nullptr, (uint64_t)0, n_live);
+}
+
+}
diff --git a/stratum-dsp_amd/csrc/kernels.hpp b/stratum-dsp_amd/csrc/kernels.hpp
--- a/stratum-dsp_amd/csrc/kernels.hpp
+++ b/stratum-dsp_amd/csrc/kernels.hpp
@@ -303,18 +303,22 @@
                       float fd, float* chroma, float* energy, hipStream_t st);
 bool mask_band_ok(int margin, float power);
 void launch_mask_band(float* mags, int stride, int B, const uint64_t* frame_pfx, const int* tracks, int n_items,
-                      float power, int st_lo, int st_hi, float* part, uint64_t total, hipStream_t st,
-                      bool outside = false);
+                      float power, int st_lo, int st_hi, float* part, uint64_t total, hipStream_t st);
+void launch_mask_outside(float* mags, int stride, int B, const uint64_t* frame_pfx, const int* tracks, int n_items,
+                         float power, int st_lo, int st_hi, hipStream_t st, const int* n_live = nullptr);
 void launch_hpcp_band(const float* mags, const uint64_t* frame_pfx, const uint64_t* tile_pfx, const int* tracks,
                       int n_items, uint64_t n_tiles, const HpcpParams& P, const HarmEntry* harm, const float* part,
                       uint64_t total, float* chroma, float* energy, float* edel, hipStream_t st);
 void launch_hpcp(const float* mags, const uint64_t* frame_pfx, const uint64_t* tile_pfx, const int* tracks,
                  int n_items, uint64_t n_tiles, const HpcpParams& P, const HarmEntry* harm, float* chroma,
-                 float* energy, hipStream_t st);
+                 float* energy, hipStream_t st, const uint64_t* n_tiles_live = nullptr);
 void launch_key_vote(const int* tracks, int n_items, const uint64_t* frame_pfx, float* chroma_raw,
                      const float* energy, float* chroma_s, float* weights, float* seg_scratch, const uint64_t* seg_off,
                      const float* tmpl, const KeyParams& P, KeyOut* out, hipStream_t st, KeyDbg* dbg = nullptr,
-                     const float* edel = nullptr, float* wdel = nullptr, bool alone = false);
+                     const float* edel = nullptr, float* wdel = nullptr, bool alone = false, const int* n_live = nullptr);
+void launch_key_near_select(const int* tracks, int n, const KeyOut* out, const uint64_t* frame_pfx,
+                            const uint64_t* seg_pfx, int* sel, int* count, uint64_t* tile_pfx, uint64_t* seg_off,
+                            hipStream_t st);
 void launch_synth(float* out, uint64_t n_tracks, uint64_t len, uint32_t sr, const float* bpm, const int* key,
                   uint64_t seed0, hipStream_t st);
 void launch_synth_normalize(float* out, uint64_t n_tracks, uint64_t len, unsigned int* peak_bits, hipStream_t st);
diff --git a/stratum-dsp_amd/csrc/pipeline.hip b/stratum-dsp_amd/csrc/pipeline.hip
--- a/stratum-dsp_amd/csrc/pipeline.hip
+++ b/stratum-dsp_amd/csrc/pipeline.hip
@@ -13,7 +13,7 @@
 }
 
 Pipeline::Pipeline(DeviceCtx& d, const sdsp_config& cfg, uint32_t sr, int stages, bool exact_energy, bool key_only,
-                   bool nested, bool probe)
+                   bool probe)
     : c_(d),
       d_(d),
       cfg_(cfg),
@@ -21,14 +21,14 @@
       bpm_only_(stages == SDSP_STAGES_BPM_ONLY),
       exact_energy_(exact_energy),
       key_only_(key_only),
-      nested_(nested || probe),
+      probe_(probe),
       fs_((int)std::min<uint64_t>(cfg.frame_size, STFT_GEN_MAX)),
       nb_(fs_ / 2 + 1),
       s2_(base_stride(fs_)),
       kfs_((int)std::min<uint64_t>(key_fft(cfg), STFT_GEN_MAX)),
       khop_((int)std::min<uint64_t>(std::max<uint64_t>(key_hop(cfg), 1), INT32_MAX)),
       ks_(base_stride(kfs_)) {
-    if (nested_) c_.pre = probe ? "D." : "X.";
+    if (probe_) c_.pre = "D.";
 }
 
 void Pipeline::run(const float* d_samples, const std::vector<uint64_t>& in_off, const std::vector<uint64_t>& n_raw,
@@ -54,8 +54,7 @@
         if (hipMemGetInfo(&fr, &tot) == hipSuccess) {
             double held = 0;
             for (auto& kv : d_.bufs)
-                if (kv.first.compare(0, c_.pre.size(), c_.pre) == 0 && (!c_.pre.empty() || kv.first.compare(0, 2, "X.") != 0))
-                    held += (double)kv.second->bytes;
+                if (kv.first.compare(0, c_.pre.size(), c_.pre) == 0) held += (double)kv.second->bytes;
             budget = std::max(4e9, ((double)fr + held) * 0.80 / 1.125);
         }
         if (const double gb = test_hooks().hbm_budget_gb.load(); gb > 0.0) budget = std::max(1.0, gb) * 1e9;
@@ -102,12 +101,12 @@
     last_sub_ = true;
     flush();
     last_sub_ = false;
-    rerun_tail(finish_key(res, true), res);
+    finish_key(res);
     times_.total_ms = std::chrono::duration<double, std::milli>(std::chrono::steady_clock::now() - t0).count();
     times_.key_reruns = reruns_;
     times_.rerun_ms = rerun_ms_;
     d_.last = times_;
-    if (!exact_energy_ && !nested_) d_.last_tail_reruns = tail_reruns_;
+    if (!exact_energy_ && !probe_) d_.last_tail_reruns = tail_reruns_;
 }
 
 void Pipeline::loudness_prepass(const float* d_samples, const std::vector<uint64_t>& in_off,
@@ -200,7 +199,7 @@
     }
     const Beats bt = beat_grid(bin, bo, on, tp);
     tm.mark(5);
-    std::vector<KeyOut> kout = join_key(d_samples, in_off, n_raw, f, kl, htr, res);
+    std::vector<KeyOut> kout = join_key(f, kl, htr, res);
     const ResultsHost rh = download_results(bt, bin, bo);
     htr("D down");
     if (cfg_.enable_key_beat_synchronous && !cfg_.enable_key_log_frequency && !kl.K.empty()) {
diff --git a/stratum-dsp_amd/csrc/pipeline.hpp b/stratum-dsp_amd/csrc/pipeline.hpp
--- a/stratum-dsp_amd/csrc/pipeline.hpp
+++ b/stratum-dsp_amd/csrc/pipeline.hpp
@@ -235,24 +235,23 @@
 void print_debug(const sdsp_config& c, const TrackDbg& d);
 
 struct KeyTail {
-    bool ok = false;
     float* mags8 = nullptr;
     uint64_t* d_kpfx = nullptr;
     std::vector<uint64_t> kpfx{0}, kseg{0};
-    float* d_part = nullptr;
     uint64_t total8 = 0;
     int st_lo = 0, st_hi = -1, B8 = 0;
     HpcpParams hp{};
     const HarmEntry* d_ht = nullptr;
-    float *d_chroma = nullptr, *d_energy = nullptr, *d_cs = nullptr, *d_w = nullptr, *d_sscr = nullptr;
+    float *d_chroma = nullptr, *d_energy = nullptr;
     const float* d_tpl = nullptr;
     KeyParams kp{};
 };
 struct KeyPending {
-    std::unique_ptr<Timers> kt;
-    KeyOut* d_kout = nullptr;
+    std::unique_ptr<Timers> kt, kt_b;
+    KeyOut *d_kout = nullptr, *d_kout2 = nullptr;
     std::vector<size_t> at;
-    KeyTail tail;
+    bool halves = false;
+    uint64_t split_row = 0;
 };
 struct KeyCond {
     HpcpParams hp{};
@@ -282,6 +281,10 @@
     KeyDbg* d_kdbg = nullptr;
     KeyTail tail;
     std::unique_ptr<Timers> kt;
+    bool halves = false;
+    std::unique_ptr<Timers> kt_b;
+    KeyOut* d_kout2 = nullptr;
+    uint64_t split_row = 0;
 };
 struct Hpss {
     float *d_P0 = nullptr, *d_hpe = nullptr, *d_hfmax = nullptr;
@@ -324,7 +327,7 @@
 class Pipeline {
    public:
     Pipeline(DeviceCtx& d, const sdsp_config& cfg, uint32_t sr, int stages = SDSP_STAGES_FULL, bool exact_energy = false,
-             bool key_only = false, bool nested = false, bool probe = false);
+             bool key_only = false, bool probe = false);
     void debug_tempo_stages(const float* host_mags, const uint64_t* frames, uint64_t n_tracks, int hop,
                             sdsp_debug_tempo_out* out);
     void debug_key_stages(const float* host_mags, const uint64_t* frames, uint64_t n_tracks, int mode, float* masked,
@@ -341,7 +344,7 @@
     bool bpm_only_ = false;
     bool exact_energy_ = false;
     bool key_only_ = false;
-    bool nested_ = false;
+    bool probe_ = false;
     bool last_sub_ = false;
     uint64_t reruns_ = 0;
     uint64_t tail_reruns_ = 0;
@@ -352,7 +355,6 @@
     std::vector<float> loud_gain_;
     std::vector<int> loud_stat_;
     std::unique_ptr<KeyPending> key_pending_;
-    std::unique_ptr<KeyPending> tail_;
     int sb_parity_ = 0;
 
     bool tg_on() const { return !cfg_.force_legacy_bpm; }
@@ -393,19 +395,18 @@
     void legacy_select(const Front& f, const TempoPassIn& bin, const Onsets& on, Tempo& tp, std::vector<TrackRes>& res);
 
     KeyLaunch launch_key(const float* d_samples, const TempoPassIn& bin);
+    void launch_key_halves(KeyLaunch& kl, const float* d_samples, const std::string& EP, const uint64_t* d_ksrc,
+                           const float* d_kgain, const uint64_t* d_kseg);
+    HpcpParams key_hpcp_params() const;
     KeyCond key_condition(const std::string& EP, float* mags8, const std::vector<uint64_t>& kpfx,
                           const std::vector<uint64_t>& ktile, uint64_t* d_kpfx, uint64_t* d_ktile, int* d_kid,
                           hipStream_t st2, Timers& kt);
     void join_key_only(KeyLaunch& kl, const Front& f, std::vector<TrackRes>& res);
-    std::vector<KeyOut> join_key(const float* d_samples, const std::vector<uint64_t>& in_off,
-                                 const std::vector<uint64_t>& n_raw, const Front& f, KeyLaunch& kl, HostTrace& htr,
-                                 std::vector<TrackRes>& res);
-    std::vector<size_t> finish_key(std::vector<TrackRes>& res, bool keep_tail = false);
-    void rerun_near(const float* d_samples, const std::vector<uint64_t>& in_off, const std::vector<uint64_t>& n_raw,
-                    const std::vector<size_t>& near, std::vector<TrackRes>& res);
-    void rerun_tail(const std::vector<size_t>& near, std::vector<TrackRes>& res);
+    std::vector<KeyOut> join_key(const Front& f, KeyLaunch& kl, HostTrace& htr, std::vector<TrackRes>& res);
+    void finish_key(std::vector<TrackRes>& res);
     void tail_buffers(KeyTail& t, const KeyCond& kc, float* mags8, uint64_t* d_kpfx, uint64_t total8) const;
-    void tail_exact(const KeyTail& t, const int* d_sel, int n, const uint64_t* d_tiles, uint64_t n_tiles, hipStream_t st);
+    void tail_exact(const KeyTail& t, const int* d_sel, int n, const uint64_t* d_tiles, uint64_t n_tiles, hipStream_t st,
+                    const int* n_live = nullptr, const uint64_t* tiles_live = nullptr);
     void beat_sync_revote(const KeyLaunch& kl, const ResultsHost& rh, std::vector<KeyOut>& kout);
 
     void debug_base(const TempoPassIn& bin, const TempoPassOut& bo, const std::vector<TempoEst>& best,
diff --git a/stratum-dsp_amd/csrc/pipeline_abi.hip b/stratum-dsp_amd/csrc/pipeline_abi.hip
--- a/stratum-dsp_amd/csrc/pipeline_abi.hip
+++ b/stratum-dsp_amd/csrc/pipeline_abi.hip
@@ -288,7 +288,7 @@
     for (uint64_t t = 0; t < n_tracks; t++)
         if (frames[t] == 0 || frames[t] > (1u << 24)) return SDSP_ERR_INVALID_INPUT;
     return run_stage_probe("sdsp_debug_tempo_stages", device, [&](DeviceCtx& d) {
-        Pipeline p(d, *cfg, sample_rate, SDSP_STAGES_FULL, false, false, false, true);
+        Pipeline p(d, *cfg, sample_rate, SDSP_STAGES_FULL, false, false, true);
         p.debug_tempo_stages(host_mags, frames, n_tracks, (int)hop, out);
     });
 }
@@ -302,7 +302,7 @@
     for (uint64_t t = 0; t < n_tracks; t++)
         if (frames[t] == 0 || frames[t] > (1u << 24)) return SDSP_ERR_INVALID_INPUT;
     return run_stage_probe("sdsp_debug_key_stages", device, [&](DeviceCtx& d) {
-        Pipeline p(d, *cfg, sample_rate, SDSP_STAGES_FULL, mode == 2, false, false, true);
+        Pipeline p(d, *cfg, sample_rate, SDSP_STAGES_FULL, mode == 2, false, true);
         p.debug_key_stages(host_mags, frames, n_tracks, mode, masked, chroma, energy, edel, info);
     });
 }
diff --git a/stratum-dsp_amd/csrc/pipeline_key.hip b/stratum-dsp_amd/csrc/pipeline_key.hip
--- a/stratum-dsp_amd/csrc/pipeline_key.hip
+++ b/stratum-dsp_amd/csrc/pipeline_key.hip
@@ -30,7 +30,7 @@
     kt.init(d_);
     sb_parity_ ^= 1;
     const std::string EP = sb_parity_ ? "E1." : "E0.";
-    kl.serial_streams = nested_ || test_hooks().serial_streams.load() != 0;
+    kl.serial_streams = probe_ || test_hooks().serial_streams.load() != 0;
     hipStream_t st2 = kl.serial_streams ? st : d_.stream2;
     hipStream_t st3 = kl.serial_streams ? st : d_.stream3;
     if (NK == 0) return kl;
@@ -39,8 +39,6 @@
     t.d_kpfx = c_.up(EP + "kpfx", t.kpfx);
     kl.d_ktile = c_.up(EP + "ktile", kl.ktile);
     uint64_t* d_kseg = c_.up(EP + "kseg", t.kseg);
-    const std::vector<uint64_t> kstr = stft_strips(t.kpfx);
-    uint64_t* d_kstr = c_.up(EP + "kstrip", kstr);
     uint64_t* d_ksrc = c_.up(EP + "ksrc", ksrc);
     float* d_kgain = c_.up(EP + "kgain", kgain);
     std::vector<int> kid((size_t)NK);
@@ -48,6 +46,16 @@
     kl.d_kid = c_.up(EP + "kid", kid);
     FftTables& t8 = d_.tables(KFS, true);
     t.mags8 = c_.dev<float>("E.mags8", total8 * ks_);
+    times_.stft8192_frames += total8;
+    times_.stft8192_bytes += key_in_bytes + 4.0 * (double)total8 * (double)B8;
+    kl.halves = !kl.serial_streams && !dbg_on() && !key_only_ && !exact_energy_ &&
+                test_hooks().no_key_defer.load() == 0 && key_energy_blocked(cfg_, sr_);
+    if (kl.halves) {
+        launch_key_halves(kl, d_samples, EP, d_ksrc, d_kgain, d_kseg);
+        return kl;
+    }
+    const std::vector<uint64_t> kstr = stft_strips(t.kpfx);
+    uint64_t* d_kstr = c_.up(EP + "kstrip", kstr);
     kt.mark(7);
     SDSP_HIP_CHECK(hipStreamWaitEvent(st2, kt.ev[7], 0));
     kt.mark(0, st2);
@@ -67,13 +75,6 @@
     float* d_w = c_.dev<float>("E.weights", total8);
     float* d_sscr = c_.dev<float>("E.segscr", std::max<uint64_t>(t.kseg.back(), 1));
     kl.d_kout = c_.dev<KeyOut>(EP + "kout", (size_t)NK);
-    if (kc.band && kc.d_ht) {
-        t.ok = true;
-        tail_buffers(t, kc, t.mags8, t.d_kpfx, total8);
-        t.d_cs = d_cs;
-        t.d_w = d_w;
-        t.d_sscr = d_sscr;
-    }
     kt.mark(8);
     kt.mark(11, st2);
     SDSP_HIP_CHECK(hipStreamWaitEvent(st3, kt.ev[8], 0));
@@ -81,14 +82,129 @@
     kl.d_kdbg = dbg_on() ? c_.dev<KeyDbg>(EP + "kdbg", (size_t)NK) : nullptr;
     float* d_wdel = kc.d_edel ? c_.dev<float>("E.wdel", total8) : nullptr;
     launch_key_vote(kl.d_kid, NK, t.d_kpfx, kc.d_chroma, kc.d_energy, d_cs, d_w, d_sscr, d_kseg, t.d_tpl, t.kp,
-                    kl.d_kout, st3, kl.d_kdbg, kc.d_edel, d_wdel, last_sub_ || nested_ || key_only_);
+                    kl.d_kout, st3, kl.d_kdbg, kc.d_edel, d_wdel, last_sub_ || probe_ || key_only_);
     SDSP_HIP_CHECK(hipGetLastError());
     kt.mark(2, st3);
-    if (!nested_) SDSP_HIP_CHECK(hipEventRecord(d_.vote_done, st3));
+    if (!probe_) SDSP_HIP_CHECK(hipEventRecord(d_.vote_done, st3));
     times_.stft8192_launches += 1;
-    times_.stft8192_frames += total8;
-    times_.stft8192_bytes += key_in_bytes + 4.0 * (double)total8 * (double)B8;
     return kl;
+}
+
+void Pipeline::launch_key_halves(KeyLaunch& kl, const float* d_samples, const std::string& EP, const uint64_t* d_ksrc,
+                                 const float* d_kgain, const uint64_t* d_kseg) {
+    KeyTail& t = kl.tail;
+    hipStream_t st2 = d_.stream2, st3 = d_.stream3;
+    const int NK = (int)kl.K.size(), KFS = kfs_, B8 = KFS / 2 + 1;
+    const uint64_t total8 = t.kpfx.back();
+    int ka = 1;
+    for (int k = 2; k < NK; k++) {
+        const uint64_t half = total8 / 2, a = t.kpfx[(size_t)ka], b = t.kpfx[(size_t)k];
+        if ((b > half ? b - half : half - b) < (a > half ? a - half : half - a)) ka = k;
+    }
+    const KeyPending* prev = key_pending_ && key_pending_->halves ? key_pending_.get() : nullptr;
+    if (prev && prev->kt_b && t.kpfx[(size_t)ka] > prev->split_row) {
+        int kb = ka;
+        while (kb > 1 && t.kpfx[(size_t)kb] > prev->split_row) kb--;
+        if (t.kpfx[(size_t)kb] <= prev->split_row && t.kpfx[(size_t)kb] >= total8 / 8 * 3) ka = kb;
+    }
+    const int h0[3] = {0, ka, NK};
+    kl.split_row = t.kpfx[(size_t)ka];
+    std::vector<uint64_t> fpfx[2], strips[2], tiles[2];
+    uint64_t *d_fpfx[2] = {}, *d_strips[2] = {}, *d_tiles[2] = {};
+    for (int h = 0; h < 2; h++) {
+        for (int k = h0[h]; k <= h0[h + 1]; k++) {
+            fpfx[h].push_back(t.kpfx[(size_t)k] - t.kpfx[(size_t)h0[h]]);
+            tiles[h].push_back(kl.ktile[(size_t)k] - kl.ktile[(size_t)h0[h]]);
+        }
+        if (h0[h + 1] == h0[h]) continue;
+        strips[h] = stft_strips(fpfx[h]);
+        const std::string X = EP + (h ? "b." : "a.");
+        d_fpfx[h] = c_.up(X + "fpfx", fpfx[h]);
+        d_strips[h] = c_.up(X + "kstrip", strips[h]);
+        d_tiles[h] = c_.up(X + "ktile", tiles[h]);
+    }
+    FftTables& t8 = d_.tables(KFS, true);
+    KeyCond kc;
+    HpcpParams& hp = kc.hp = key_hpcp_params();
+    kc.band = true;
+    kc.st_lo = hp.pk_lo - 1;
+    kc.st_hi = hp.pk_hi + 1;
+    kc.d_part = c_.dev<float>("E.kpart", total8 * (uint64_t)((B8 + 63) / 64));
+    kc.d_chroma = c_.dev<float>("E.chroma", total8 * 12);
+    kc.d_energy = c_.dev<float>("E.energy", total8);
+    kc.d_edel = c_.dev<float>("E.edel", total8);
+    kc.d_ht = c_.up(EP + "harm", harm_table(B8, sr_, KFS, cfg_.soft_mapping_sigma, hp.hmax, cfg_.key_hpcp_harmonic_decay));
+    tail_buffers(t, kc, t.mags8, t.d_kpfx, total8);
+    std::vector<float> tpl(576);
+    key_templates(tpl.data());
+    t.d_tpl = c_.up(EP + "tpl", tpl);
+    t.kp.near_check = 1;
+    t.kp.cert_fixed = test_hooks().key_cert_fixed.load();
+    KeyParams kx = t.kp;
+    kx.near_check = 0;
+    float* d_cs = c_.dev<float>("E.chroma_s", total8 * 12);
+    float* d_w = c_.dev<float>("E.weights", total8);
+    float* d_sscr = c_.dev<float>("E.segscr", std::max<uint64_t>(t.kseg.back(), 1));
+    float* d_wdel = c_.dev<float>("E.wdel", total8);
+    uint32_t* d_redo = c_.dev<uint32_t>("E.redo", total8 + 1);
+    kl.d_kout = c_.dev<KeyOut>(EP + "kout", (size_t)NK);
+    kl.d_kout2 = c_.dev<KeyOut>(EP + "kout2", (size_t)NK);
+    int* d_rsel = c_.dev<int>("E.rsel", (size_t)NK);
+    int* d_rcnt = c_.dev<int>("E.rcnt", 1);
+    uint64_t* d_rtile = c_.dev<uint64_t>("E.rtile", (size_t)NK + 1);
+    uint64_t* d_rseg = c_.dev<uint64_t>("E.rseg", (size_t)NK);
+    kl.kt->mark(7);
+    SDSP_HIP_CHECK(hipStreamWaitEvent(st2, kl.kt->ev[7], 0));
+    for (int h = 0; h < 2; h++) {
+        const int a = h0[h], n = h0[h + 1] - h0[h];
+        if (n == 0) continue;
+        if (h) {
+            kl.kt_b.reset(new Timers());
+            kl.kt_b->init(d_);
+        }
+        Timers& tm = h ? *kl.kt_b : *kl.kt;
+        if (prev) {
+            hipEvent_t ra = prev->kt->ev[3], rb = prev->kt_b ? prev->kt_b->ev[3] : nullptr;
+            if (h == 0) SDSP_HIP_CHECK(hipStreamWaitEvent(st2, ra, 0));
+            if (rb && (h == 1 || t.kpfx[(size_t)ka] > prev->split_row)) SDSP_HIP_CHECK(hipStreamWaitEvent(st2, rb, 0));
+        }
+        tm.mark(0, st2);
+        launch_stft(KFS, false, d_samples, d_fpfx[h], n, fpfx[h].back(), d_ksrc + a, d_kgain + a, khop_,
+                    t8.window.as<float>(), stft_twp(t8, KFS, false), stft_rtp(t8, KFS, false), t.mags8, t.d_kpfx + a, ks_,
+                    nullptr, st2, d_strips[h], strips[h].back(), d_redo);
+        SDSP_HIP_CHECK(hipGetLastError());
+        tm.mark(1, st2);
+        launch_mask_band(t.mags8, ks_, B8, t.d_kpfx, kl.d_kid + a, n, cfg_.key_harmonic_mask_power, kc.st_lo, kc.st_hi,
+                         kc.d_part, total8, st2);
+        launch_hpcp_band(t.mags8, t.d_kpfx, d_tiles[h], kl.d_kid + a, n, tiles[h].back(), hp, kc.d_ht, kc.d_part, total8,
+                         kc.d_chroma, kc.d_energy, kc.d_edel, st2);
+        SDSP_HIP_CHECK(hipGetLastError());
+        tm.mark(11, st2);
+        SDSP_HIP_CHECK(hipStreamWaitEvent(st3, tm.ev[11], 0));
+        const bool alone = last_sub_ && h0[h + 1] == NK;
+        launch_key_vote(kl.d_kid + a, n, t.d_kpfx, kc.d_chroma, kc.d_energy, d_cs, d_w, d_sscr, d_kseg + a, t.d_tpl, t.kp,
+                        kl.d_kout, st3, nullptr, kc.d_edel, d_wdel, alone);
+        SDSP_HIP_CHECK(hipGetLastError());
+        tm.mark(2, st3);
+        launch_key_near_select(kl.d_kid + a, n, kl.d_kout, t.d_kpfx, d_kseg, d_rsel, d_rcnt, d_rtile, d_rseg, st3);
+        tail_exact(t, d_rsel, n, d_rtile, tiles[h].back(), st3, d_rcnt, d_rtile + n);
+        launch_key_vote(d_rsel, n, t.d_kpfx, kc.d_chroma, kc.d_energy, d_cs, d_w, d_sscr, d_rseg, t.d_tpl, kx, kl.d_kout2,
+                        st3, nullptr, nullptr, nullptr, alone, d_rcnt);
+        SDSP_HIP_CHECK(hipGetLastError());
+        tm.mark(3, st3);
+    }
+    times_.stft8192_launches += 1;
+}
+
+HpcpParams Pipeline::key_hpcp_params() const {
+    HpcpParams hp{};
+    hp.B = kfs_ / 2 + 1;
+    hp.stride = ks_;
+    key_peak_band(cfg_, sr_, &hp.pk_lo, &hp.pk_hi);
+    hp.K = (int)std::max<uint64_t>(cfg_.key_hpcp_peaks_per_frame, 1);
+    hp.hmax = (int)std::max<uint64_t>(cfg_.key_hpcp_num_harmonics, 1);
+    hp.p = sd_clampf(cfg_.key_hpcp_mag_power, 0.05f, 1.0f);
+    return hp;
 }
 
 KeyCond Pipeline::key_condition(const std::string& EP, float* mags8, const std::vector<uint64_t>& kpfx,
@@ -104,13 +220,7 @@
     const bool tuned = cfg_.enable_key_tuning_compensation && !use_log;
     const bool whiten = cfg_.enable_key_hpcp_whitening && cfg_.key_hpcp_whitening_smooth_bins >= 3;
     KeyCond kc;
-    HpcpParams& hp = kc.hp;
-    hp.B = B8;
-    hp.stride = ks_;
-    key_peak_band(cfg_, sr_, &hp.pk_lo, &hp.pk_hi);
-    hp.K = (int)std::max<uint64_t>(cfg_.key_hpcp_peaks_per_frame, 1);
-    hp.hmax = (int)std::max<uint64_t>(cfg_.key_hpcp_num_harmonics, 1);
-    hp.p = sd_clampf(cfg_.key_hpcp_mag_power, 0.05f, 1.0f);
+    HpcpParams& hp = kc.hp = key_hpcp_params();
     const bool blocked = key_energy_blocked(cfg_, sr_);
     const bool band = kc.band = blocked && !exact_energy_;
     float* d_part = kc.d_part = blocked ? c_.dev<float>("E.kpart", total8 * (uint64_t)((B8 + 63) / 64)) : nullptr;
@@ -154,7 +264,7 @@
     float* d_chroma = kc.d_chroma = c_.dev<float>("E.chroma", total8 * 12);
     float* d_energy = kc.d_energy = c_.dev<float>("E.energy", total8);
     float* d_edel = nullptr;
-    if (!nested_) SDSP_HIP_CHECK(hipStreamWaitEvent(st2, d_.vote_done, 0));
+    if (!probe_) SDSP_HIP_CHECK(hipStreamWaitEvent(st2, d_.vote_done, 0));
     if (use_log) {
         const ChromaParams cp = chroma_params(cfg_, sr_, 1, B8, fres8, ks_);
         launch_chroma(1, mags8, d_kpfx, d_ktile, d_kid, NK, ktile.back(), cp, nullptr, d_chroma, d_energy, st2);
@@ -191,10 +301,8 @@
         if (ko[k].ok) set_key_fields(res[f.slot[(size_t)kl.K[k]]], ko[k]);
 }
 
-std::vector<KeyOut> Pipeline::join_key(const float* d_samples, const std::vector<uint64_t>& in_off,
-                                       const std::vector<uint64_t>& n_raw, const Front& f, KeyLaunch& kl,
-                                       HostTrace& htr, std::vector<TrackRes>& res) {
-    rerun_near(d_samples, in_off, n_raw, finish_key(res), res);
+std::vector<KeyOut> Pipeline::join_key(const Front& f, KeyLaunch& kl, HostTrace& htr, std::vector<TrackRes>& res) {
+    finish_key(res);
     std::vector<KeyOut> kout;
     const size_t NK = kl.K.size();
     const bool beat_sync = cfg_.enable_key_beat_synchronous && !cfg_.enable_key_log_frequency;
@@ -203,9 +311,12 @@
     if (defer_key) {
         key_pending_.reset(new KeyPending());
         key_pending_->kt = std::move(kl.kt);
+        key_pending_->kt_b = std::move(kl.kt_b);
         key_pending_->d_kout = kl.d_kout;
+        key_pending_->d_kout2 = kl.d_kout2;
+        key_pending_->halves = kl.halves;
+        key_pending_->split_row = kl.split_row;
         for (int i : kl.K) key_pending_->at.push_back(f.slot[(size_t)i]);
-        key_pending_->tail = std::move(kl.tail);
     } else if (NK > 0) {
         SDSP_HIP_CHECK(hipStreamWaitEvent(d_.stream, kl.kt->ev[2], 0));
         kout = c_.down(kl.d_kout, NK);
@@ -216,110 +327,54 @@
     return kout;
 }
 
-std::vector<size_t> Pipeline::finish_key(std::vector<TrackRes>& res, bool keep_tail) {
-    std::vector<size_t> near;
-    if (!key_pending_) return near;
+void Pipeline::finish_key(std::vector<TrackRes>& res) {
+    if (!key_pending_) return;
     std::unique_ptr<KeyPending> kp = std::move(key_pending_);
-    SDSP_HIP_CHECK(hipStreamWaitEvent(d_.stream, kp->kt->ev[2], 0));
+    Timers& last = kp->kt_b ? *kp->kt_b : *kp->kt;
+    SDSP_HIP_CHECK(hipStreamWaitEvent(d_.stream, last.ev[kp->halves ? 3 : 2], 0));
     const std::vector<KeyOut> kout = c_.down(kp->d_kout, kp->at.size());
+    std::vector<KeyOut> kout2;
+    if (kp->halves) kout2 = c_.down(kp->d_kout2, kp->at.size());
+    uint64_t n_rerun = 0;
     for (size_t k = 0; k < kp->at.size(); k++) {
         TrackRes& r = res[kp->at[k]];
         const KeyOut& ko = kout[k];
         if (!ko.ok) continue;
         set_key_fields(r, ko);
         r.key_near = ko.near;
-        if (ko.near) near.push_back(kp->at[k]);
-    }
-    times_.stft8192_ms += kp->kt->ms(0, 1);
-    times_.key_ms += kp->kt->ms(1, 2);
-    if (keep_tail && kp->tail.ok) tail_ = std::move(kp);
-    return near;
-}
-
-void Pipeline::rerun_tail(const std::vector<size_t>& near_all, std::vector<TrackRes>& res) {
-    std::unique_ptr<KeyPending> kp = std::move(tail_);
-    if (near_all.empty() || !kp || exact_energy_ || nested_) return;
-    const KeyTail& t = kp->tail;
-    const auto t0 = std::chrono::steady_clock::now();
-    std::vector<size_t> near;
-    for (size_t i : near_all)
-        if (res[i].status == SDSP_OK) near.push_back(i);
-    if (near.empty()) return;
-    std::vector<int> sel;
-    for (size_t i : near)
-        for (size_t k = 0; k < kp->at.size(); k++)
-            if (kp->at[k] == i) sel.push_back((int)k);
-    if (sel.size() != near.size()) throw HipError("rerun_tail: a near track is not in the last sub-batch");
-    const int n = (int)sel.size();
-    std::vector<uint64_t> tp(1, 0), sp(1, 0);
-    for (int k : sel) {
-        const uint64_t F = t.kpfx[(size_t)k + 1] - t.kpfx[(size_t)k];
-        tp.push_back(tp.back() + (F + HP_FRAMES - 1) / HP_FRAMES);
-        sp.push_back(sp.back() + (t.kseg[(size_t)k + 1] - t.kseg[(size_t)k]));
-    }
-    hipStream_t st = d_.stream;
-    int* d_sel = c_.up("E.tail_sel", sel);
-    uint64_t* d_tp = c_.up("E.tail_tile", tp);
-    uint64_t* d_sp = c_.up("E.tail_seg", sp);
-    tail_exact(t, d_sel, n, d_tp, tp.back(), st);
-    KeyParams kx = t.kp;
-    kx.near_check = 0;
-    launch_key_vote(d_sel, n, t.d_kpfx, t.d_chroma, t.d_energy, t.d_cs, t.d_w, t.d_sscr, d_sp, t.d_tpl, kx, kp->d_kout,
-                    st, nullptr, nullptr, nullptr, true);
-    SDSP_HIP_CHECK(hipGetLastError());
-    const std::vector<KeyOut> ko = c_.down(kp->d_kout, kp->at.size());
-    for (int j = 0; j < n; j++) {
-        TrackRes& r = res[near[(size_t)j]];
-        const KeyOut& o = ko[(size_t)sel[(size_t)j]];
-        if (!o.ok) {
+        if (!ko.near || !kp->halves) continue;
+        if (r.status != SDSP_OK) continue;
+        r.key_rerun = true;
+        n_rerun++;
+        if (!kout2[k].ok) {
             r.status = SDSP_ERR_PROCESSING;
             r.err = "Processing error: key certification rerun failed (no key from the exact energies)";
-            r.key_rerun = true;
             continue;
         }
-        set_key_fields(r, o);
-        r.key_rerun = true;
-    }
-    reruns_ += (uint64_t)n;
-    tail_reruns_ += (uint64_t)n;
-    rerun_ms_ += std::chrono::duration<double, std::milli>(std::chrono::steady_clock::now() - t0).count();
+        set_key_fields(r, kout2[k]);
+    }
+    reruns_ += n_rerun;
+    tail_reruns_ += n_rerun;
+    for (Timers* tm : {kp->kt.get(), kp->kt_b.get()}) {
+        if (!tm) continue;
+        times_.stft8192_ms += tm->ms(0, 1);
+        times_.key_ms += tm->ms(1, 2);
+        if (kp->halves) rerun_ms_ += tm->ms(2, 3);
+    }
 }
 
 void Pipeline::tail_exact(const KeyTail& t, const int* d_sel, int n, const uint64_t* d_tiles, uint64_t n_tiles,
-                          hipStream_t st) {
-    launch_mask_band(t.mags8, ks_, t.B8, t.d_kpfx, d_sel, n, cfg_.key_harmonic_mask_power, t.st_lo, t.st_hi, t.d_part,
-                     t.total8, st, true);
-    SDSP_HIP_CHECK(hipGetLastError());
-    launch_hpcp(t.mags8, t.d_kpfx, d_tiles, d_sel, n, n_tiles, t.hp, t.d_ht, t.d_chroma, t.d_energy, st);
-    SDSP_HIP_CHECK(hipGetLastError());
-}
-
-void Pipeline::rerun_near(const float* d_samples, const std::vector<uint64_t>& in_off, const std::vector<uint64_t>& n_raw,
-                          const std::vector<size_t>& near, std::vector<TrackRes>& res) {
-    if (near.empty() || exact_energy_ || nested_) return;
-    std::vector<uint64_t> o2, l2;
-    for (size_t i : near) o2.push_back(in_off[i]), l2.push_back(n_raw[i]);
-    std::vector<TrackRes> r2;
-    Pipeline px(d_, cfg_, sr_, SDSP_STAGES_FULL, true, true, true);
-    px.run(d_samples, o2, l2, r2);
-    for (size_t j = 0; j < near.size(); j++) {
-        TrackRes& r = res[near[j]];
-        if (r2[j].status != SDSP_OK) {
-            r.status = SDSP_ERR_PROCESSING;
-            r.err = "Processing error: key certification rerun failed (" + r2[j].err + ")";
-            continue;
-        }
-        set_key_fields(r, r2[j]);
-        r.key_rerun = true;
-    }
-    reruns_ += near.size();
-    rerun_ms_ += d_.last.total_ms;
+                          hipStream_t st, const int* n_live, const uint64_t* tiles_live) {
+    launch_mask_outside(t.mags8, ks_, t.B8, t.d_kpfx, d_sel, n, cfg_.key_harmonic_mask_power, t.st_lo, t.st_hi, st,
+                        n_live);
+    SDSP_HIP_CHECK(hipGetLastError());
+    launch_hpcp(t.mags8, t.d_kpfx, d_tiles, d_sel, n, n_tiles, t.hp, t.d_ht, t.d_chroma, t.d_energy, st, tiles_live);
+    SDSP_HIP_CHECK(hipGetLastError());
 }
 
 void Pipeline::tail_buffers(KeyTail& t, const KeyCond& kc, float* mags8, uint64_t* d_kpfx, uint64_t total8) const {
     t.mags8 = mags8;
     t.d_kpfx = d_kpfx;
-    t.d_part = kc.d_part;
     t.total8 = total8;
     t.st_lo = kc.st_lo;
     t.st_hi = kc.st_hi;
```

New measurement: 3015. No clear change (-0.0%).
